# nikisalli/nightmare_rl

Measured on AMD Instinct MI355X. Metric: env-steps/sec at N parallel Nightmare-v3 envs, 1/2/4/8 MI355X, higher is better.
Workload: dtype f32; 1 GPU; 4096 Nightmare-v3 envs per GPU, random-action rollout U(-1,1)^18, full step(): 2 x 8 ms substeps (18-DoF dynamics + floor contact, PGS x3 + noslip x4) + obs/reward/termination/reset; envs_per_gpu=4096, decimation=2

## Files before the change

### nightmare_rl_amd/csrc/nm_core.h

```cpp
#pragma once
#include <type_traits>
#include <stddef.h>

#include "simt.h"

#ifdef NM_MEASURE
#define NM_ABLATE(mask) (mask)
#else
#define NM_ABLATE(mask) 0
#endif
namespace nm {
using namespace simt;

constexpr int kNQ = 25, kNV = 24, kNU = 18, kNLEG = 6, kNCOL = 7, kNSENS = 13, kNOBS = 66, kNREW = 16;
constexpr int kLinkN = 25;
constexpr int kLegN = 3 * kLinkN;
constexpr int kBaseN = 10;
constexpr int kColN = 24;
constexpr int kMaxCon = 16;
constexpr int kMaxRow = 4 * kMaxCon;
constexpr int kMaxConBig = 44;
constexpr int kBigSlots = (4 * kMaxConBig + NM_WAVE - 1) / NM_WAVE;
constexpr int kJRow = 16;
enum { R_ACTION_RATE, R_ANG_VEL_XY, R_BASE_HEIGHT, R_BODY_CONTACT, R_DEFAULT_POS, R_DOF_ACC, R_DOF_VEL, R_FEET_AIR_TIME, R_FEET_CONTACT,
       R_LIN_VEL_Z, R_ORIENTATION, R_STAND_STILL, R_TORQUES, R_TRACK_ANG, R_TRACK_LIN, R_TERMINATION };

template <class real> struct Model {
  const real* hullv;
  const real* hullnv;
  real legc[kNLEG * kLegN];
  real basec[kBaseN];
  real colc[kNCOL * kColN];
  real footc[kNLEG * 4];
  real qpos0[kNQ];
  int maxnbr;
  int link_rot_id[3];
  real total_mass;
  real h, kv, ctrl_max, grav, mu;
  real solref_K, solref_B, si_d0, si_dmax, si_width, si_mid, si_power;
  real pgs_scale, pgs_tol, noslip_tol, tol_planemesh;
  int pgs_iters, noslip_iters, mpr_iters;
  real mpr_tol;
  real dt, p_gain, clip_obs, obs_lin, obs_ang, obs_dofpos, obs_dofvel, max_lin_x, max_ang, term_force, sigma, max_ep_len, default_pos[3];
  float action_scale, clip_actions;
  int resample_every;
  real rew_scale[kNREW];
  real ep_len_s;
  int rew_extra;
  int tibia_mode, body_mode;
  int collide_batch_min;
  real tibia_max, body_max, base_h_target, max_contact_force;
};

template <class real> struct Args {
  int N;
  int rec_env;
  uint64_t seed;
  int64_t env_offset;
  real *qpos, *qvel, *qwarm;
  real *dofpos, *dofvel, *act, *cmd, *epsum;
  real* feetair;
  int* feetflags;
  int64_t* eplen;
  uint32_t* rngctr;
  int* hullcache;
  const float* actions;
  const real* cmd_u;
  float *obs, *rew, *timeout_now;
  float* ret_acc;
  int64_t* done;
  real* stat_sum;
  int* stat_cnt;
  int* wave_done;
  int *nto, *to_list;
  int *nprev, *to_prev;
  unsigned long long* to_owner;
  float *ep_stats, *time_outs;
  long long* counters;
  real* dbg;
  int nsub;
  int nxcd;
  int physics_only;
  int ablate;
  const real* noise_vec;
  const real* noise_u;
  uint64_t noise_step;
  real* rec;
  const real* envp;
};
constexpr int kTicketGroup = 64, kTicketStride = 32, kTicketTop = 0;
constexpr uint64_t kNoiseKey = 0x4E4F495345ull;
constexpr uint64_t kEnvParamKey = 0x454E5650ull;
constexpr int EP_MU = 0, EP_PGAIN = 1, EP_KV = 2, kEnvP = 4, kEnvPS = 3;
constexpr int kBodyP = 20, BP_IPOS = 0, BP_I6 = 3, BP_MASS = 9, BP_TOTAL = 10, BP_INVW = 11, BP_PGS = 18;
constexpr uint64_t kPayloadKey = 0x5041594C4Full;
constexpr int kLatH = 3, kLatP = 1 + kLatH * 18;
constexpr uint64_t kLatencyKey = 0x4C4154454Eull;
template <class real> NM_FN int* lat_delay(const Args<real>& A) {
  return reinterpret_cast<int*>(const_cast<real*>(A.envp) + (size_t)A.N * (kEnvP + kBodyP));
}
template <class real> NM_FN float* lat_hist(const Args<real>& A) { return reinterpret_cast<float*>(lat_delay(A) + A.N); }
constexpr int kDbgN = 256;

template <class real> struct Sh {
  real qpos[kNQ];
  real envp[kEnvPS];
  real qvel[24], warm[24], ctrl[20];
  real Rb[9], wv[6];
  real anc[kNU * 3], axs[kNU * 3];
  real colR[kNCOL * 9], colp[kNCOL * 3];
  real Minv[kNLEG * 6], W[kNLEG * 18], Lb[15], Dbi[6];
  real MinvH[kNLEG * 6], WH[kNLEG * 18], LbH[15], DbiH[6];
  real qas[24], qfs[24], qfc[24];
  real vv[24];
  real sens[16], cvb[6];
  real bh[2];
  real mbb[36], sc[36];
  real legtmp[kNLEG * 66];
  NM_FN real* cpos() { return legtmp; }
  NM_FN real* cnrm() { return legtmp + 3 * kMaxConBig; }
  NM_FN real* cdist() { return legtmp + 6 * kMaxConBig; }
  NM_FN int* cleg() { return reinterpret_cast<int*>(legtmp + 7 * kMaxConBig); }
  NM_FN int* cleg1() { return reinterpret_cast<int*>(legtmp + 8 * kMaxConBig); }
  real efc_f[kMaxRow];
#ifdef NM_DEBUG_SOLVER
  real dbg_b[kMaxRow], dbg_a[kMaxRow], dbg_f0[kMaxRow];
#endif
  int ncon, nwarn, it_pgs, it_noslip, anypair;
  int nhop;
  int ntog;
  real eact[kNU], epact[kNU], epdv[kNU];
  real ecmd[4], eepsum[kNREW];
  int eplen_lo, eplen_hi;
  unsigned ectr;
  int cstart[8], ccnt[8];
  real sink[NM_WAVE];
  int hcache[8];
};

static_assert(kNLEG * 66 >= 9 * kMaxConBig, "contact list must fit the leg staging area");
static_assert(offsetof(Sh<float>, qvel) == 28 * sizeof(float) && offsetof(Sh<double>, qvel) == 28 * sizeof(double), "qpos + envp keep the 28 words qpos had");
template <class real, int G> struct ShW {
  Sh<real> e[G];
  alignas(16) real jrow[kMaxRow * kJRow];
};
template <class real, int G> struct ShWB {
  ShW<real, G> w;
  real body[G * kBodyP];
};
template <class real, int G> NM_FN real* body_rows(ShW<real, G>& w) { return reinterpret_cast<ShWB<real, G>*>(&w)->body; }
template <class real, int G, int EP> struct ShWSel {
  typedef ShW<real, G> type;
  static NM_FN ShW<real, G>& images(type& s) { return s; }
};
template <class real, int G> struct ShWSel<real, G, 2> {
  typedef ShWB<real, G> type;
  static NM_FN ShW<real, G>& images(type& s) { return s.w; }
};
template <class real, int G> struct ShWL {
  ShWB<real, G> b;
  real late[G * 18];
  int rsw[G];
};
template <class real, int G> NM_FN ShWL<real, G>& lat_rows(ShW<real, G>& w) { return *reinterpret_cast<ShWL<real, G>*>(&w); }
template <class real, int G> struct ShWSel<real, G, 3> {
  typedef ShWL<real, G> type;
  static NM_FN ShW<real, G>& images(type& s) { return s.b.w; }
};
#define NM_OFS(field) ((int)(offsetof(Sh<real>, field) / sizeof(real)))
#define NM_IOFS(field) ((int)(offsetof(Sh<real>, field) / sizeof(int)))

template <int EP, class real> NM_FN real env_mu(const Sh<real>& sh, const Model<real>& M) {
  if constexpr (EP != 0) return sh.envp[EP_MU]; else return M.mu;
}
template <int EP, class real> struct BodyRef {
  NM_FN BodyRef() {}
  NM_FN explicit BodyRef(const real*) {}
};
template <class real> struct BodyRef<2, real> {
  const real* p;
  NM_FN BodyRef() : p(nullptr) {}
  NM_FN explicit BodyRef(const real* q) : p(q) {}
};
template <class real> struct BodyRef<3, real> {
  const real* p;
  NM_FN BodyRef() : p(nullptr) {}
  NM_FN explicit BodyRef(const real* q) : p(q) {}
};
template <int EP, class real> NM_FN V<real> body_invw(const BodyRef<EP, real>& b, const Model<real>& M, const V<int>& g) {
  if constexpr (EP >= 2) return ldsv(b.p, g + BP_INVW); else return ldsv(M.colc, g * kColN + 4);
}
template <int EP, class real> NM_FN real body_pgs(const BodyRef<EP, real>& b, const Model<real>& M) {
  if constexpr (EP >= 2) return b.p[BP_PGS]; else return M.pgs_scale;
}

template <class A, class B, class C> NM_FN void cross3(A* r, const B* a, const C* b) {
  A x = a[1] * b[2] - a[2] * b[1], y = a[2] * b[0] - a[0] * b[2], z = a[0] * b[1] - a[1] * b[0];
  r[0] = x; r[1] = y; r[2] = z;
}
template <class A, class B, class C> NM_FN A dot3(const B* a, const C* b) { return a[0] * b[0] + a[1] * b[1] + a[2] * b[2]; }
template <class A, class B, class C> NM_FN void matvec3(A* r, const B* m, const C* v) {
  A x = m[0] * v[0] + m[1] * v[1] + m[2] * v[2], y = m[3] * v[0] + m[4] * v[1] + m[5] * v[2], z = m[6] * v[0] + m[7] * v[1] + m[8] * v[2];
  r[0] = x; r[1] = y; r[2] = z;
}
template <class A, class B, class C> NM_FN void matvec3_fma(A* r, const B* m, const C* v) {
  A x = vfma(A(m[2]), A(v[2]), vfma(A(m[1]), A(v[1]), A(m[0]) * A(v[0])));
  A y = vfma(A(m[5]), A(v[2]), vfma(A(m[4]), A(v[1]), A(m[3]) * A(v[0])));
  A z = vfma(A(m[8]), A(v[2]), vfma(A(m[7]), A(v[1]), A(m[6]) * A(v[0])));
  r[0] = x; r[1] = y; r[2] = z;
}
template <class A, class B, class C> NM_FN void matmul3(A* r, const B* a, const C* b) {
#pragma unroll
  for (int i = 0; i < 3; i++)
#pragma unroll
    for (int j = 0; j < 3; j++) r[3 * i + j] = a[3 * i] * b[j] + a[3 * i + 1] * b[3 + j] + a[3 * i + 2] * b[6 + j];
}
template <class A, class B, class C> NM_FN void inert_mul(A* r, const B* i, const C* v) {
  r[0] = i[0] * v[0] + i[3] * v[1] + i[4] * v[2] - i[8] * v[4] + i[7] * v[5];
  r[1] = i[3] * v[0] + i[1] * v[1] + i[5] * v[2] + i[8] * v[3] - i[6] * v[5];
  r[2] = i[4] * v[0] + i[5] * v[1] + i[2] * v[2] - i[7] * v[3] + i[6] * v[4];
  r[3] = i[8] * v[1] - i[7] * v[2] + i[9] * v[3];
  r[4] = i[6] * v[2] - i[8] * v[0] + i[9] * v[4];
  r[5] = i[7] * v[0] - i[6] * v[1] + i[9] * v[5];
}
template <class A, class B, class C> NM_FN void cross_motion(A* r, const B* vel, const C* v) {
  A a[3], b[3], c[3];
  cross3(a, vel, v); cross3(b, vel, v + 3); cross3(c, vel + 3, v);
  r[0] = a[0]; r[1] = a[1]; r[2] = a[2]; r[3] = b[0] + c[0]; r[4] = b[1] + c[1]; r[5] = b[2] + c[2];
}
template <class A, class B, class C> NM_FN void cross_force(A* r, const B* vel, const C* f) {
  A a[3], b[3], c[3];
  cross3(a, vel, f); cross3(b, vel + 3, f + 3); cross3(c, vel, f + 3);
  r[0] = a[0] + b[0]; r[1] = a[1] + b[1]; r[2] = a[2] + b[2]; r[3] = c[0]; r[4] = c[1]; r[5] = c[2];
}
template <class A, class B, class C> NM_FN A dot6(const B* a, const C* b) {
  return a[0] * b[0] + a[1] * b[1] + a[2] * b[2] + a[3] * b[3] + a[4] * b[4] + a[5] * b[5];
}
template <class real> NM_FN real lanesum6(const V<real>& x) {
  return ((rdlane(x, 0) + rdlane(x, 1)) + (rdlane(x, 2) + rdlane(x, 3))) + (rdlane(x, 4) + rdlane(x, 5));
}
template <class X, class real> NM_FN void spatial_inertia(X* I10, const X* R, const X* Ib, const X* d, X m, real) {
  X T[9];
#pragma unroll
  for (int i = 0; i < 3; i++) {
    T[3 * i + 0] = R[3 * i] * Ib[0] + R[3 * i + 1] * Ib[3] + R[3 * i + 2] * Ib[4];
    T[3 * i + 1] = R[3 * i] * Ib[3] + R[3 * i + 1] * Ib[1] + R[3 * i + 2] * Ib[5];
    T[3 * i + 2] = R[3 * i] * Ib[4] + R[3 * i + 1] * Ib[5] + R[3 * i + 2] * Ib[2];
  }
  X xx = T[0] * R[0] + T[1] * R[1] + T[2] * R[2], yy = T[3] * R[3] + T[4] * R[4] + T[5] * R[5], zz = T[6] * R[6] + T[7] * R[7] + T[8] * R[8];
  X xy = T[0] * R[3] + T[1] * R[4] + T[2] * R[5], xz = T[0] * R[6] + T[1] * R[7] + T[2] * R[8], yz = T[3] * R[6] + T[4] * R[7] + T[5] * R[8];
  I10[0] = xx + m * (d[1] * d[1] + d[2] * d[2]);
  I10[1] = yy + m * (d[0] * d[0] + d[2] * d[2]);
  I10[2] = zz + m * (d[0] * d[0] + d[1] * d[1]);
  I10[3] = xy - m * d[0] * d[1];
  I10[4] = xz - m * d[0] * d[2];
  I10[5] = yz - m * d[1] * d[2];
  I10[6] = m * d[0]; I10[7] = m * d[1]; I10[8] = m * d[2];
  I10[9] = m;
}
template <class X, class real> NM_FN void ldl3(X* r, const X* a, real one) {
  X i2 = vrcp(a[5]);
  X l21 = a[4] * i2, l20 = a[2] * i2;
  X m11 = a[3] - l21 * a[4], m01 = a[1] - l21 * a[2], m00 = a[0] - l20 * a[2];
  X i1 = vrcp(m11);
  X l10 = m01 * i1;
  X d0 = m00 - l10 * m01;
  r[0] = l21; r[1] = l20; r[2] = l10; r[3] = i2; r[4] = i1; r[5] = vrcp(d0);
}
template <class X, class Y> NM_FN void ldl3_solve(X* x, const X* f, const Y* y) {
  X y2 = y[2];
  X y1 = y[1] - f[0] * y2;
  X y0 = y[0] - f[1] * y2 - f[2] * y1;
  X x0 = y0 * f[5];
  X x1 = y1 * f[4] - f[2] * x0;
  x[2] = y2 * f[3] - f[0] * x1 - f[1] * x0;
  x[1] = x1; x[0] = x0;
}
template <class X, class real, class Acc> NM_FN void ldl6(Acc S, X* L, X* Dinv, real one) {
  X Lf[36], D[6];
#pragma unroll
  for (int j = 0; j < 6; j++) {
    X d = S(j, j);
#pragma unroll
    for (int k = 0; k < j; k++) d = d - Lf[6 * j + k] * Lf[6 * j + k] * D[k];
    D[j] = d;
    X di = vrcp(d);
    Dinv[j] = di;
#pragma unroll
    for (int i = j + 1; i < 6; i++) {
      X s = S(j, i);
#pragma unroll
      for (int k = 0; k < j; k++) s = s - Lf[6 * i + k] * Lf[6 * j + k] * D[k];
      Lf[6 * i + j] = s * di;
    }
  }
  int n = 0;
#pragma unroll
  for (int i = 1; i < 6; i++)
#pragma unroll
    for (int j = 0; j < i; j++) L[n++] = Lf[6 * i + j];
}
template <class LT, class X> NM_FN void ldl6_solve(const LT* L, const LT* Dinv, X* x) {
  int n = 0;
#pragma unroll
  for (int i = 1; i < 6; i++)
#pragma unroll
    for (int j = 0; j < i; j++) x[i] = x[i] - L[n++] * x[j];
#pragma unroll
  for (int i = 0; i < 6; i++) x[i] = x[i] * Dinv[i];
#pragma unroll
  for (int i = 5; i >= 1; i--) {
    n = i * (i - 1) / 2;
#pragma unroll
    for (int j = 0; j < i; j++) x[j] = x[j] - L[n + j] * x[i];
  }
}

NM_HDFN uint32_t rand_u24_bits(uint64_t seed, uint64_t genv, uint32_t ctr) {
  uint64_t x = seed + 0x9E3779B97F4A7C15ull * (genv + 1) + 0xD1B54A32D192ED03ull * (uint64_t)ctr;
  x ^= x >> 30; x *= 0xBF58476D1CE4E5B9ull;
  x ^= x >> 27; x *= 0x94D049BB133111EBull;
  x ^= x >> 31;
  return (uint32_t)(x >> 40);
}

#ifndef NM_EMUL
template <class T> NM_FN void nm_consume(T x) { asm volatile("" ::"v"(x) : "memory"); }
#endif

#if defined(NM_STAMPS) && !defined(NM_EMUL)
__device__ unsigned long long g_stamps[16];
NM_FN void nm_stamp(int k) {
  __shared__ unsigned long long tl, acc[16];
#ifdef NM_STAMPS_B
  asm volatile("s_waitcnt vmcnt(0) lgkmcnt(0)" ::: "memory");
#endif
  unsigned long long n = __builtin_amdgcn_s_memtime();
  if (NM_TID == 0) {
    if (k < 0) for (int i = 0; i < 16; i++) acc[i] = 0;
    else acc[k] += n - tl;
    if (k == 10) for (int i = 0; i < 16; i++) atomicAdd(&g_stamps[i], acc[i]);
    tl = n;
  }
}
#else
NM_FN void nm_stamp(int) {}
#endif
#ifdef NM_STAMPS_B
#define NM_ESTAMP(k)
#define NM_BSTAMP(k) nm_stamp(k)
#else
#define NM_ESTAMP(k) nm_stamp(k)
#define NM_BSTAMP(k)
#endif

constexpr int kLinkTmp = 22;

template <class real> NM_FN V<real> legsum(const V<real>& x, const VB& isleg) {
  return gsum8(sel(isleg, x, V<real>(real(0))));
}

template <int EP, class real, int G> NM_FN void stage_smooth(ShW<real, G>& w, const Model<real>& M, bool last) {
  typedef V<real> vr;
  real* lds = reinterpret_cast<real*>(&w.e[0]);
  static_assert((G & (G - 1)) == 0 && 2 * G <= 8, "lane groups: G envs x 2 factorisations");
  const V<int> lane0 = opaque_lane();
  const V<int> sub = lane0 & 7, grp = lane0 >> 3;
  const V<int> leg = vmin(sub, V<int>(5)), eo = (grp & (G - 1)) * (int)(sizeof(Sh<real>) / sizeof(real));
  const VB pass1 = (grp & G) != 0;
  const VB isleg = sub < V<int>(6);
#define LDG(field, i) ldsv(lds, eo + (NM_OFS(field) + (i)))
  const V<int> bo = (grp & (G - 1)) * kBodyP + (int)(sizeof(ShW<real, G>) / sizeof(real));
#define LDB(i) ldsv(lds, bo + (i))
  const VB st_all = VB(true), st_leg = VB(true);
#define STG(field, i, val) stsv(lds, eo + (NM_OFS(field) + (i)), val, st_all)
#define LDL(field, idx) ldsv(lds, eo + (idx) + NM_OFS(field))
#define STL(field, idx, val) stsv(lds, eo + (idx) + NM_OFS(field), val, st_leg)
  const V<int> slot = leg * (3 * kLinkTmp);

  vr Rb[9];
  {
    vr qw = LDG(qpos, 3), qx = LDG(qpos, 4), qy = LDG(qpos, 5), qz = LDG(qpos, 6);
    {
      const vr in_ = vrcp(vsqrt(qw * qw + qx * qx + qy * qy + qz * qz));
      qw = qw * in_; qx = qx * in_; qy = qy * in_; qz = qz * in_;
      STG(qpos, 3, qw); STG(qpos, 4, qx); STG(qpos, 5, qy); STG(qpos, 6, qz);
    }
    vr q00 = qw * qw, q01 = qw * qx, q02 = qw * qy, q03 = qw * qz, q11 = qx * qx, q12 = qx * qy, q13 = qx * qz, q22 = qy * qy,
       q23 = qy * qz, q33 = qz * qz;
    Rb[0] = q00 + q11 - q22 - q33; Rb[4] = q00 - q11 + q22 - q33; Rb[8] = q00 - q11 - q22 + q33;
    Rb[1] = real(2) * (q12 - q03); Rb[2] = real(2) * (q13 + q02); Rb[3] = real(2) * (q12 + q03);
    Rb[5] = real(2) * (q23 - q01); Rb[6] = real(2) * (q13 - q02); Rb[7] = real(2) * (q23 + q01);
  }
  vr vb[6], ab[6];
  {
    vr wl[3] = {LDG(qvel, 3), LDG(qvel, 4), LDG(qvel, 5)};
    matvec3(vb, Rb, wl);
    vb[3] = LDG(qvel, 0); vb[4] = LDG(qvel, 1); vb[5] = LDG(qvel, 2);
    vr t[3];
    cross3(t, vb + 3, vb);
    ab[0] = ab[1] = ab[2] = vr(real(0));
    ab[3] = t[0]; ab[4] = t[1]; ab[5] = t[2] + M.grav;
  }
#pragma unroll
  for (int j = 0; j < 9; j++) { STG(colR, j, Rb[j]); STG(Rb, j, Rb[j]); }
#pragma unroll
// ... 2306 lines not shown
    sh.eplen_hi = (int)(ep >> 32);
    sh.ectr = ctr_in;
    if constexpr (EP == 3) {
      const int nsub = A.nsub;
      const int k = (dl >= nsub ? 1 : 0) + (dl >= 2 * nsub ? 1 : 0) + (dl >= 3 * nsub ? 1 : 0), r = dl - k * nsub;
      const V<float> fl = k == 0 ? af : (k == 1 ? h0 : (k == 2 ? h1 : h2));
      const V<float> fe = r > 0 ? (k == 0 ? h0 : (k == 1 ? h1 : h2)) : fl;
      stsv(sh.ctrl, lane, ((vcvt<real>(fe) - defp) - dofpos_old) * p_gain, l18);
      stsv(late, lane, ((vcvt<real>(fl) - defp) - dofpos_old) * p_gain, l18);
      *rsw = r;
      float* hist = lat_hist(A);
      const VB st = l18 & VB(live);
      gstv(hist, lane + (env * (kLatH * kNU) + 2 * kNU), h1, st);
      gstv(hist, lane + (env * (kLatH * kNU) + kNU), h0, st);
      gstv(hist, lane + env * (kLatH * kNU), af, st);
    } else
    stsv(sh.ctrl, lane, ((act - defp) - dofpos_old) * p_gain, l18);
  } else {
    wave_sync();
    stsv(sh.ctrl, lane, ((act - defp) - ldsv(sh.qpos, l18c + 7)) * p_gain, l18);
    if constexpr (EP == 3) *rsw = 0;
  }
  stsv(sh.eact, lane, act, l18); stsv(sh.epact, lane, prev_act, l18); stsv(sh.epdv, lane, prev_dofvel, l18);
  wave_sync();
}

template <class real> NM_FN void env_debug(Sh<real>& sh, const Args<real>& A, int env, int dropped) {
  const V<int> lane = opaque_lane();
  {
    real* dbg = A.dbg + (size_t)env * kDbgN;
    gstv(dbg, lane, ldsv(sh.qas, sel(lane < 24, lane, V<int>(0))), lane < 24);
    gstv(dbg, lane + 24, ldsv(sh.qfs, sel(lane < 24, lane, V<int>(0))), lane < 24);
    gstv(dbg, lane + 48, ldsv(sh.qfc, sel(lane < 24, lane, V<int>(0))), lane < 24);
    gstv(dbg, lane + 72, ldsv(sh.sens, sel(lane < 13, lane, V<int>(0))), lane < 13);
    gstv(dbg, lane + 88, ldsv(sh.cvb, sel(lane < 6, lane, V<int>(0))), lane < 6);
    gstv(dbg, lane + 96, ldsv(sh.cdist(), sel(lane < kMaxCon, lane, V<int>(0))), lane < kMaxCon);
    gstv(dbg, lane + 112, ldsv(sh.cpos(), sel(lane < 3 * kMaxCon, lane, V<int>(0))), lane < 3 * kMaxCon);
    gstv(dbg, V<int>(160), to_real<real>(sh.ncon), lane == 0);
    gstv(dbg, V<int>(161), to_real<real>(sh.nwarn), lane == 0);
    gstv(dbg, V<int>(162), to_real<real>(dropped), lane == 0);
    gstv(dbg, lane + 165, ldsv(sh.cnrm(), sel(lane < 6, lane, V<int>(0))), lane < 6);
    gstv(dbg, lane + 150, to_real<real>(ldsv(sh.hcache, sel(lane < 7, lane, V<int>(0)))), lane < 7);
    gstv(dbg, V<int>(158), to_real<real>(sh.hcache[7]), lane == 0);
    gstv(dbg, V<int>(159), to_real<real>(sh.nhop), lane == 0);
    gstv(dbg, V<int>(157), to_real<real>(sh.anypair), lane == 0);
    gstv(dbg, V<int>(156), to_real<real>(sh.ntog), lane == 0);
    gstv(dbg, V<int>(163), to_real<real>(sh.it_pgs), lane == 0);
    gstv(dbg, V<int>(164), to_real<real>(sh.it_noslip), lane == 0);
    gstv(dbg, lane + 176, ldsv(sh.efc_f, lane), lane < kMaxRow);
#ifdef NM_DEBUG_SOLVER
    gstv(dbg, lane + 240, ldsv(sh.dbg_b, sel(lane < 4, lane, V<int>(0))), lane < 4);
    gstv(dbg, lane + 244, ldsv(sh.dbg_a, sel(lane < 4, lane, V<int>(0))), lane < 4);
    gstv(dbg, lane + 248, ldsv(sh.dbg_f0, sel(lane < 4, lane, V<int>(0))), lane < 4);
#endif
  }
}

template <class real> NM_FN void env_finish(Sh<real>& sh, const Model<real>& M, const Args<real>& A, int env,
                                            int dropped, bool live) {
  typedef V<real> vr;
  if (!live) return;
  const V<int> lane = opaque_lane();
  const VB l18 = lane < kNU;
  const V<int> l18c = sel(l18, lane, V<int>(0));
  const vr act = ldsv(sh.eact, l18c), prev_act = ldsv(sh.epact, l18c), prev_dofvel = ldsv(sh.epdv, l18c);
  vr defp;
  {
    V<int> m3 = lane % 3;
    defp = sel(m3 == 1, vr(M.default_pos[1]), sel(m3 == 0, vr(M.default_pos[0]), vr(M.default_pos[2])));
  }
  {
    const V<int> hc = ldsv(sh.hcache, sel(lane < 8, lane, V<int>(0)));
    const vr q = ldsv(sh.qpos, sel(lane < kNQ, lane, V<int>(0))), v = ldsv(sh.qvel, sel(lane < kNV, lane, V<int>(0))),
             w = ldsv(sh.warm, sel(lane < kNV, lane, V<int>(0)));
    gstv(A.hullcache, lane + env * 8, hc, lane < 8);
    gstv(A.qpos, lane + env * kNQ, q, lane < kNQ);
    gstv(A.qvel, lane + env * kNV, v, lane < kNV);
    gstv(A.qwarm, lane + env * kNV, w, lane < kNV);
  }
  if (A.rec && env == A.rec_env) {
    gstv(A.rec, lane, ldsv(sh.qpos, sel(lane < kNQ, lane, V<int>(0))), lane < kNQ);
    gstv(A.rec, lane + kNQ, ldsv(sh.qvel, sel(lane < kNV, lane, V<int>(0))), lane < kNV);
    gstv(A.rec, V<int>(kNQ + kNV), to_real<real>(sh.nwarn), lane == 0);
  }
  if (A.dbg) env_debug(sh, A, env, dropped);
  if ((dropped | sh.nwarn) && A.stat_cnt) {
#ifdef NM_EMUL
    A.stat_cnt[1] += dropped; A.stat_cnt[2] += sh.nwarn;
#else
    if (NM_TID == 0) { nm_consume(atomicAdd(A.stat_cnt + 1, dropped)); nm_consume(atomicAdd(A.stat_cnt + 2, sh.nwarn)); }
#endif
  }
  if (A.physics_only) return;
  NM_ESTAMP(11);

  int64_t eplen = (((int64_t)sh.eplen_hi << 32) | (int64_t)(uint32_t)sh.eplen_lo) + 1;
  real bq[4] = {sh.qpos[3], -sh.qpos[4], -sh.qpos[5], -sh.qpos[6]};
  auto rot = [&](real* r, const real* v) {
    real tx = real(2) * (bq[2] * v[2] - bq[3] * v[1]), ty = real(2) * (bq[3] * v[0] - bq[1] * v[2]), tz = real(2) * (bq[1] * v[1] - bq[2] * v[0]);
    r[0] = v[0] + bq[0] * tx + (bq[2] * tz - bq[3] * ty);
    r[1] = v[1] + bq[0] * ty + (bq[3] * tx - bq[1] * tz);
    r[2] = v[2] + bq[0] * tz + (bq[1] * ty - bq[2] * tx);
  };
  real blv[3], bav[3], pg[3];
  {
    real lin[3] = {sh.cvb[3], sh.cvb[4], sh.cvb[5]}, ang[3] = {sh.cvb[0], sh.cvb[1], sh.cvb[2]}, gv[3] = {real(0), real(0), -M.grav};
    rot(blv, lin); rot(bav, ang); rot(pg, gv);
  }
  vr dofpos = ldsv(sh.qpos, l18c + 7), dofvel = ldsv(sh.qvel, l18c + 6);
  real tib[6], feet[6], body = sh.sens[12];
#pragma unroll
  for (int l = 0; l < 6; l++) {
    feet[l] = sh.sens[6 + l];
    tib[l] = feet[l] == real(0) ? sh.sens[l] : real(0);
  }
  real cmd[3] = {sh.ecmd[0], sh.ecmd[1], sh.ecmd[2]};
  uint32_t ctr = sh.ectr;
  auto resample = [&](int which) {
    real ux, uy;
    if (A.cmd_u) { ux = gld1(A.cmd_u, env * 4 + 2 * which); uy = gld1(A.cmd_u, env * 4 + 2 * which + 1); }
    else {
      ux = (real)rand_u24_bits(A.seed, (uint64_t)(A.env_offset + env), ctr) * real(1.0 / 16777216.0);
      uy = (real)rand_u24_bits(A.seed, (uint64_t)(A.env_offset + env), ctr + 1) * real(1.0 / 16777216.0);
      ctr += 2;
    }
    cmd[0] = ux * real(2) * M.max_lin_x - M.max_lin_x;
    cmd[1] = real(0);
    cmd[2] = uy * real(2) * M.max_ang - M.max_ang;
    real keep = vsqrt(cmd[0] * cmd[0] + cmd[1] * cmd[1]) > real(0.02) ? real(1) : real(0);
    cmd[0] = cmd[0] * keep; cmd[1] = cmd[1] * keep;
  };
  {
    bool due;
    if (eplen >= 0 && eplen < (1 << 22)) {
      const int e32 = (int)eplen, R = M.resample_every;
      const int q = (int)((float)e32 / (float)R);
      const int r = e32 - q * R;
      due = r == 0 || r == R || r == -R;
    } else due = eplen % M.resample_every == 0;
    if (due) resample(0);
  }
  bool time_out = (real)eplen > M.max_ep_len;
  bool reset = time_out;
  {
    real fm = feet[0];
#pragma unroll
    for (int l = 1; l < 6; l++) fm = vmax(fm, feet[l]);
    reset = reset | (fm > M.term_force);
    if ((M.tibia_mode == 2) | (M.body_mode == 2)) {
      real tm = tib[0];
#pragma unroll
      for (int l = 1; l < 6; l++) tm = vmax(tm, tib[l]);
      if (M.tibia_mode == 2) reset = reset | (tm > M.tibia_max);
      if (M.body_mode == 2) reset = reset | (body > M.body_max);
    }
    real nrm = vsqrt(pg[0] * pg[0] + pg[1] * pg[1] + pg[2] * pg[2]);
    if (sizeof(real) == 8) reset = reset | (vacos(-pg[2] / nrm) > real(1.0471975511965976));
    else reset = reset | (-pg[2] / nrm <= real(0.5));
  }
  NM_ESTAMP(12);
  vr epsum[1];
  V<int> l8c = sel(lane < kNREW, lane, V<int>(0));
  epsum[0] = ldsv(sh.eepsum, l8c);
  if (reset) {
    gstv(A.qpos, lane + env * kNQ, ldsv(M.qpos0, sel(lane < kNQ, lane, V<int>(0))), lane < kNQ);
    gstv(A.qvel, lane + env * kNV, real(0), lane < kNV);
    resample(1);
    eplen = 0;
#ifdef NM_EMUL
    for (int k = 0; k < kNREW; k++) A.stat_sum[k] += epsum[0].v[k];
    A.stat_cnt[0] += 1;
#else
    if (NM_TID < kNREW) nm_consume(atomicAdd(A.stat_sum + NM_TID, epsum[0]));
    if (NM_TID == 0) {
      nm_consume(atomicAdd(A.stat_cnt, 1));
      if (time_out && A.to_list) nm_consume(atomicExch(A.to_list + atomicAdd(A.nto, 1), env));
    }
#endif
    epsum[0] = vr(real(0));
  }
  NM_ESTAMP(13);
  real rt[kNREW];
#pragma unroll
  for (int k = 0; k < kNREW; k++) rt[k] = real(0);
  {
    vr da = prev_act - act;
    rt[R_ACTION_RATE] = wsum<real>(sel(l18, da * da, vr(real(0)))) * M.rew_scale[R_ACTION_RATE];
    real sumt = ((tib[0] + tib[1]) + (tib[2] + tib[3])) + (tib[4] + tib[5]);
    if ((M.tibia_mode != 1) | (M.body_mode != 1)) {
      sumt = M.tibia_mode == 1 ? sumt : real(0);
      body = M.body_mode == 1 ? body : real(0);
    }
    rt[R_BODY_CONTACT] = (sumt + body) * M.rew_scale[R_BODY_CONTACT];
    vr dp = dofpos - defp;
    rt[R_DEFAULT_POS] = wsum<real>(sel(l18, dp * dp, vr(real(0)))) * M.rew_scale[R_DEFAULT_POS];
    vr acc = (dofvel - prev_dofvel) / M.dt;
    rt[R_DOF_ACC] = wsum<real>(sel(l18, acc * acc, vr(real(0)))) * M.rew_scale[R_DOF_ACC];
    rt[R_ORIENTATION] = (pg[0] * pg[0] + pg[1] * pg[1]) * M.rew_scale[R_ORIENTATION];
    real ea = (cmd[2] - bav[2]) * (cmd[2] - bav[2]);
    rt[R_TRACK_ANG] = vexp(-ea / M.sigma) * M.rew_scale[R_TRACK_ANG];
    real el = (cmd[0] - blv[0]) * (cmd[0] - blv[0]) + (cmd[1] - blv[1]) * (cmd[1] - blv[1]);
    rt[R_TRACK_LIN] = vexp(-el / M.sigma) * M.rew_scale[R_TRACK_LIN];
    rt[R_TERMINATION] = (reset && !time_out) ? M.rew_scale[R_TERMINATION] : real(0);
    if (M.rew_extra) {
      rt[R_ANG_VEL_XY] = (bav[0] * bav[0] + bav[1] * bav[1]) * M.rew_scale[R_ANG_VEL_XY];
      real dh = sh.bh[0] - M.base_h_target;
      rt[R_BASE_HEIGHT] = dh * dh * M.rew_scale[R_BASE_HEIGHT];
      rt[R_DOF_VEL] = wsum<real>(sel(l18, dofvel * dofvel, vr(real(0)))) * M.rew_scale[R_DOF_VEL];
      rt[R_LIN_VEL_Z] = blv[2] * blv[2] * M.rew_scale[R_LIN_VEL_Z];
      real still = vsqrt(cmd[0] * cmd[0] + cmd[1] * cmd[1]) < real(0.01) ? real(1) : real(0);
      rt[R_STAND_STILL] = wsum<real>(sel(l18, vabs(dp), vr(real(0)))) * still * M.rew_scale[R_STAND_STILL];
      const VB l6 = lane < kNLEG;
      const V<int> l6c = sel(l6, lane, V<int>(0));
      const vr ff = ldsv(sh.sens, l6c + 6);
      vr over = sel(ff > vr(M.max_contact_force), ff - M.max_contact_force, vr(real(0)));
      rt[R_FEET_CONTACT] = wsum<real>(sel(l6, over * over, vr(real(0)))) * M.rew_scale[R_FEET_CONTACT];
      if (M.rew_scale[R_FEET_AIR_TIME] != real(0)) {
        vr air = gldv(A.feetair, l6c + env * kNLEG);
        const V<int> fl = V<int>(gld1(A.feetflags, env));
        if (reset) air = vr(real(0));
        const VB contact = ff > vr(real(1));
        const VB filt = contact | (((fl >> l6c) & 1) != 0);
        const VB lastf = ((fl >> (l6c + kNLEG)) & 1) != 0;
        air = air + M.dt;
        air = sel(filt == lastf, air, vr(real(0)));
        const vr single = sel(air > vr(real(1)), air - real(1), vr(real(0))) + sel(air < vr(real(0.5)), real(0.5) - air, vr(real(0)));
        rt[R_FEET_AIR_TIME] = wsum<real>(sel(l6, single * single, vr(real(0)))) * M.rew_scale[R_FEET_AIR_TIME];
        gstv(A.feetair, l6c + env * kNLEG, air, l6);
        const int nf = (int)(ballot(l6 & contact) | (ballot(l6 & filt) << kNLEG));
#ifdef NM_EMUL
        A.feetflags[env] = nf;
#else
        if (NM_TID == 0) gst1(A.feetflags, env, nf);
#endif
      }
    }
  }
  real rew = real(0);
#pragma unroll
  for (int k = 0; k < kNREW; k++) rew = rew + rt[k];
  {
    vr add = vr(real(0));
#pragma unroll
    for (int k = 0; k < kNREW; k++) add = wrlane(add, rt[k], k);
    gstv(A.epsum, lane + env * kNREW, epsum[0] + add, lane < kNREW);
  }
  NM_ESTAMP(14);
  {
    real head[12] = {blv[0] * M.obs_lin, blv[1] * M.obs_lin, blv[2] * M.obs_lin, bav[0] * M.obs_ang, bav[1] * M.obs_ang, bav[2] * M.obs_ang,
                     pg[0], pg[1], pg[2], cmd[0] * M.obs_lin, cmd[1] * M.obs_lin, cmd[2] * M.obs_ang};
    vr o = vr(real(0));
#pragma unroll
    for (int k = 0; k < 12; k++) o = wrlane(o, head[k], k);
    auto put = [&](const vr& x0, const V<int>& idx, const VB& m) {
      vr x = x0;
      if (A.noise_vec) {
        auto nz = [&](int k) {
          real u = A.noise_u ? gld1(A.noise_u, (size_t)env * kNOBS + k)
                             : (real)rand_u24_bits(A.seed + kNoiseKey, (uint64_t)(A.env_offset + env), (uint32_t)(A.noise_step * kNOBS + k)) * real(1.0 / 16777216.0);
          return (real(2) * u - real(1)) * gld1(A.noise_vec, k);
        };
#ifdef NM_EMUL
        for (int i = 0; i < NM_WAVE; i++) if (m.v[i]) x.v[i] = x.v[i] + nz(idx.v[i]);
#else
        if (m) x = x + nz(idx);
#endif
      }
      vr cx = vmin(vmax(x, vr(-M.clip_obs)), vr(M.clip_obs));
#ifdef NM_EMUL
      for (int i = 0; i < NM_WAVE; i++) if (m.v[i]) A.obs[(size_t)env * kNOBS + idx.v[i]] = (float)cx.v[i];
#else
      if (m) gst1(A.obs, (size_t)env * kNOBS + idx, (float)cx);
#endif
    };
    put(o, lane, lane < 12);
    put((dofpos - defp) * M.obs_dofpos, lane + 12, l18);
    put(dofvel * M.obs_dofvel, lane + 30, l18);
    put(act, lane + 48, l18);
  }
  NM_ESTAMP(15);
  gstv(A.dofpos, lane + env * kNU, dofpos, l18);
  gstv(A.dofvel, lane + env * kNU, dofvel, l18);
  gstv(A.act, lane + env * kNU, act, l18);
  {
    vr cv = sel(lane == 0, vr(cmd[0]), sel(lane == 1, vr(cmd[1]), vr(cmd[2])));
    gstv(A.cmd, lane + env * 3, cv, lane < 3);
  }
#ifdef NM_EMUL
  const bool lane0 = true;
#else
  const bool lane0 = NM_TID == 0;
#endif
  if (lane0) {
    gst1(A.eplen, env, eplen);
    gst1(A.rngctr, env, ctr);
    gst1(A.rew, env, (float)rew);
    if (A.ret_acc) gadd1(A.ret_acc, env, (float)rew);
    gst1(A.done, env, (int64_t)(reset ? 1 : 0));
    gst1(A.timeout_now, env, time_out ? 1.0f : 0.0f);
  }
}

struct NoMid { NM_FN void operator()() const {} NM_FN void operator()(int) const {} };
template <int EP, class real, class Mid> NM_FN void env_load2(ShW<real, 2>& w, const Model<real>& M, const Args<real>& A, int wave, Mid&& mid) {
  typedef V<real> vr;
  constexpr int kSR = (int)(sizeof(Sh<real>) / sizeof(real)), kSI = (int)(sizeof(Sh<real>) / sizeof(int));
  const V<int> lane = opaque_lane();
  const V<int> h = lane >> 5, hl = lane & 31;
  const V<int> env0 = h + wave * 2;
  const V<int> env = sel(env0 < V<int>(A.N), env0, V<int>(A.N - 1));
  real* rb = reinterpret_cast<real*>(&w.e[0]);
  int* ib = reinterpret_cast<int*>(&w.e[0]);
  const V<int> ho = h * kSR, hoi = h * kSI;
  const VB l18 = hl < kNU;
  const V<int> l18c = sel(l18, hl, V<int>(0));
  const vr q_in = gldv(A.qpos, sel(hl < kNQ, hl, V<int>(0)) + env * kNQ);
  const vr v_in = gldv(A.qvel, sel(hl < kNV, hl, V<int>(0)) + env * kNV);
  const vr w_in = gldv(A.qwarm, sel(hl < kNV, hl, V<int>(0)) + env * kNV);
  const V<int> hc_in = gldv(A.hullcache, sel(hl < 8, hl, V<int>(0)) + env * 8);
  const V<float> a_in = gldv(A.actions, l18c + env * kNU);
  vr envp_in = vr(real(0));
  if constexpr (EP != 0) envp_in = gldv(A.envp, sel(hl < kEnvP, hl, V<int>(0)) + env * kEnvP);
  vr body_in = vr(real(0));
  if constexpr (EP >= 2) body_in = gldv(A.envp, sel(hl < kBodyP, hl, V<int>(0)) + (env * kBodyP + A.N * kEnvP));
  vr cmd_in = vr(real(0)), eps_in = vr(real(0)), prev_act = vr(real(0)), prev_dofvel = vr(real(0)), dofpos_old = vr(real(0));
  V<int> dl = V<int>(0);
  V<float> h0 = V<float>(0.0f), h1 = V<float>(0.0f), h2 = V<float>(0.0f);
  if constexpr (EP == 3)
    if (!A.physics_only) {
      dl = gldv(lat_delay(A), env);
      h0 = gldv(lat_hist(A), l18c + env * (kLatH * kNU));
      h1 = gldv(lat_hist(A), l18c + (env * (kLatH * kNU) + kNU));
      h2 = gldv(lat_hist(A), l18c + (env * (kLatH * kNU) + 2 * kNU));
    }
#ifndef NM_EMUL
  int64_t ep = 0;
  uint32_t ctr_in = 0;
#endif
  if (!A.physics_only) {
    cmd_in = gldv(A.cmd, sel(hl < 3, hl, V<int>(0)) + env * 3);
    eps_in = gldv(A.epsum, sel(hl < kNREW, hl, V<int>(0)) + env * kNREW);
#ifndef NM_EMUL
    ep = gld1(A.eplen, (size_t)env);
    ctr_in = gld1(A.rngctr, (size_t)env);
#endif
    prev_act = gldv(A.act, l18c + env * kNU);
    prev_dofvel = gldv(A.dofvel, l18c + env * kNU);
    dofpos_old = gldv(A.dofpos, l18c + env * kNU);
  }
  mid();
  stsv(rb, ho + (hl + NM_OFS(qpos)), q_in, hl < kNQ);
  stsv(rb, ho + (hl + NM_OFS(qvel)), v_in, hl < kNV);
  stsv(rb, ho + (hl + NM_OFS(warm)), w_in, hl < kNV);
  stsv(ib, hoi + (hl + NM_IOFS(hcache)), sel(hl == 0, hc_in & V<int>(0xffff), hc_in), hl < 8);
  nm_set_priority((rdlane(hc_in, 0) >> 16) + (rdlane(hc_in, 32) >> 16));
  w.e[0].nwarn = 0; w.e[1].nwarn = 0;
  w.e[0].nhop = 0; w.e[1].nhop = 0;
  w.e[0].ntog = 0; w.e[1].ntog = 0;
  vr p_gain = vr(M.p_gain);
  if constexpr (EP != 0) {
    stsv(rb, ho + (hl + NM_OFS(envp)), envp_in, hl < kEnvPS);
    if constexpr (EP >= 2) stsv(body_rows(w), h * kBodyP + hl, body_in, hl < kBodyP);
    p_gain = sel(h != 0, vr(rdlane(envp_in, 32 + EP_PGAIN)), vr(rdlane(envp_in, EP_PGAIN)));
  }
  V<float> af = a_in * M.action_scale;
  af = vmin(vmax(af, V<float>(-M.clip_actions)), V<float>(M.clip_actions));
  vr act;
  vr defp;
  {
    V<int> m3 = hl % 3;
    defp = sel(m3 == 1, vr(M.default_pos[1]), sel(m3 == 0, vr(M.default_pos[0]), vr(M.default_pos[2])));
  }
#ifdef NM_EMUL
  for (int i = 0; i < NM_WAVE; i++) act.v[i] = (real)af.v[i];
#else
  act = (real)af;
#endif
  if (!A.physics_only) {
    stsv(rb, ho + (hl + NM_OFS(ecmd)), cmd_in, hl < 3);
    stsv(rb, ho + (hl + NM_OFS(eepsum)), eps_in, hl < kNREW);
#ifdef NM_EMUL
    for (int hh = 0; hh < 2; hh++) {
      const int e = env.v[32 * hh];
      const int64_t ep = A.eplen[e];
      w.e[hh].eplen_lo = (int)(uint32_t)(ep & 0xffffffffll);
      w.e[hh].eplen_hi = (int)(ep >> 32);
      w.e[hh].ectr = A.rngctr[e];
    }
#else
    stsv(ib, hoi + NM_IOFS(eplen_lo), (int)(uint32_t)(ep & 0xffffffffll), hl == 0);
    stsv(ib, hoi + NM_IOFS(eplen_hi), (int)(ep >> 32), hl == 0);
    stsv(ib, hoi + NM_IOFS(ectr), (int)ctr_in, hl == 0);
#endif
    if constexpr (EP == 3) {
      const V<int> ns = V<int>(A.nsub), one = V<int>(1), zero = V<int>(0);
      const V<int> k = sel(dl >= ns, one, zero) + sel(dl >= ns + ns, one, zero) + sel(dl >= ns + ns + ns, one, zero), r = dl - k * ns;
      const V<float> fl = sel(k == zero, af, sel(k == one, h0, sel(k == V<int>(2), h1, h2)));
      const V<float> fe = sel(r > zero, sel(k == zero, h0, sel(k == one, h1, h2)), fl);
      ShWL<real, 2>& L = lat_rows(w);
      stsv(rb, ho + (hl + NM_OFS(ctrl)), ((vcvt<real>(fe) - defp) - dofpos_old) * p_gain, l18);
      stsv(L.late, h * kNU + hl, ((vcvt<real>(fl) - defp) - dofpos_old) * p_gain, l18);
      stsv(L.rsw, h, r, hl == zero);
      float* hist = lat_hist(A);
      const VB st = l18 & (env0 < V<int>(A.N));
      gstv(hist, hl + (env * (kLatH * kNU) + 2 * kNU), h1, st);
      gstv(hist, hl + (env * (kLatH * kNU) + kNU), h0, st);
      gstv(hist, hl + env * (kLatH * kNU), af, st);
    } else
    stsv(rb, ho + (hl + NM_OFS(ctrl)), ((act - defp) - dofpos_old) * p_gain, l18);
  } else {
    wave_sync();
    stsv(rb, ho + (hl + NM_OFS(ctrl)), ((act - defp) - ldsv(rb, ho + (l18c + (7 + NM_OFS(qpos))))) * p_gain, l18);
    if constexpr (EP == 3) stsv(lat_rows(w).rsw, h, V<int>(0), hl == V<int>(0));
  }
  stsv(rb, ho + (hl + NM_OFS(eact)), act, l18); stsv(rb, ho + (hl + NM_OFS(epact)), prev_act, l18); stsv(rb, ho + (hl + NM_OFS(epdv)), prev_dofvel, l18);
  wave_sync();
}

template <class real, class Pub> NM_FN void env_finish2(ShW<real, 2>& w, const Model<real>& M, const Args<real>& A, int wave, int dropped, Pub&& published) {
  typedef V<real> vr;
  constexpr int kSR = (int)(sizeof(Sh<real>) / sizeof(real)), kSI = (int)(sizeof(Sh<real>) / sizeof(int));
  const V<int> lane = opaque_lane();
  const V<int> h = lane >> 5, hl = lane & 31;
  const VB h1 = h != 0;
  const V<int> env = h + wave * 2;
  const VB live = env < V<int>(A.N);
  const V<int> envc = sel(live, env, V<int>(A.N - 1));
  const bool lives[2] = {wave * 2 < A.N, wave * 2 + 1 < A.N};
  const real* rb = reinterpret_cast<const real*>(&w.e[0]);
  const int* ib = reinterpret_cast<const int*>(&w.e[0]);
  const V<int> ho = h * kSR, hoi = h * kSI;
#define SHR(field, idx) ldsv(rb, ho + ((idx) + NM_OFS(field)))
#define SHI(field, idx) ldsv(ib, hoi + ((idx) + NM_IOFS(field)))
  const VB l18 = hl < kNU;
  const V<int> l18c = sel(l18, hl, V<int>(0));
  const vr act = SHR(eact, l18c), prev_act = SHR(epact, l18c), prev_dofvel = SHR(epdv, l18c);
  vr defp;
  {
    V<int> m3 = hl % 3;
    defp = sel(m3 == 1, vr(M.default_pos[1]), sel(m3 == 0, vr(M.default_pos[0]), vr(M.default_pos[2])));
  }
  const V<int> nwarn = SHI(nwarn, V<int>(0));
  {
    V<int> hc = SHI(hcache, sel(hl < 8, hl, V<int>(0)));
    hc = sel(hl == 0, hc | (SHI(ncon, V<int>(0)) << 16), hc);
    const vr q = SHR(qpos, sel(hl < kNQ, hl, V<int>(0))), v = SHR(qvel, sel(hl < kNV, hl, V<int>(0))), wq = SHR(warm, sel(hl < kNV, hl, V<int>(0)));
    gstv(A.hullcache, hl + env * 8, hc, live & (hl < 8));
    gstv(A.qpos, hl + env * kNQ, q, live & (hl < kNQ));
    gstv(A.qvel, hl + env * kNV, v, live & (hl < kNV));
    gstv(A.qwarm, hl + env * kNV, wq, live & (hl < kNV));
    if (A.rec) {
      const VB r = live & (env == V<int>(A.rec_env));
      gstv(A.rec, hl, q, r & (hl < kNQ));
      gstv(A.rec, hl + kNQ, v, r & (hl < kNV));
      gstv(A.rec, V<int>(kNQ + kNV), to_real<real>(nwarn), r & (hl == 0));
    }
  }
  if (A.dbg) {
    if (lives[0]) env_debug(w.e[0], A, wave * 2, dropped);
    if (lives[1]) env_debug(w.e[1], A, wave * 2 + 1, 0);
  }
  if (A.stat_cnt && (dropped != 0 || wany(live & (nwarn != 0)))) {
#ifdef NM_EMUL
    A.stat_cnt[1] += dropped;
    for (int hh = 0; hh < 2; hh++) if (lives[hh]) A.stat_cnt[2] += nwarn.v[32 * hh];
#else
    if (NM_TID == 0 && dropped) nm_consume(atomicAdd(A.stat_cnt + 1, dropped));
    if (hl == 0 && live && nwarn) nm_consume(atomicAdd(A.stat_cnt + 2, nwarn));
#endif
  }
  if (A.physics_only) return;
  if (NM_ABLATE(A.ablate) & 128) return;
  NM_ESTAMP(11);

  int64_t ep[2];
  uint32_t ctr[2];
#pragma unroll
  for (int hh = 0; hh < 2; hh++) {
    ep[hh] = (((int64_t)w.e[hh].eplen_hi << 32) | (int64_t)(uint32_t)w.e[hh].eplen_lo) + 1;
    ctr[hh] = w.e[hh].ectr;
  }
  vr bq[4] = {SHR(qpos, V<int>(3)), -SHR(qpos, V<int>(4)), -SHR(qpos, V<int>(5)), -SHR(qpos, V<int>(6))};
  auto rot = [&](vr* r, const vr* v) {
    vr tx = real(2) * (bq[2] * v[2] - bq[3] * v[1]), ty = real(2) * (bq[3] * v[0] - bq[1] * v[2]), tz = real(2) * (bq[1] * v[1] - bq[2] * v[0]);
    r[0] = v[0] + bq[0] * tx + (bq[2] * tz - bq[3] * ty);
    r[1] = v[1] + bq[0] * ty + (bq[3] * tx - bq[1] * tz);
    r[2] = v[2] + bq[0] * tz + (bq[1] * ty - bq[2] * tx);
  };
  vr blv[3], bav[3], pg[3];
  {
    vr lin[3] = {SHR(cvb, V<int>(3)), SHR(cvb, V<int>(4)), SHR(cvb, V<int>(5))}, ang[3] = {SHR(cvb, V<int>(0)), SHR(cvb, V<int>(1)), SHR(cvb, V<int>(2))};
    vr gv[3] = {vr(real(0)), vr(real(0)), vr(-M.grav)};
    rot(blv, lin); rot(bav, ang); rot(pg, gv);
  }
  vr dofpos = SHR(qpos, l18c + 7), dofvel = SHR(qvel, l18c + 6);
  vr tib[6], feet[6], body = SHR(sens, V<int>(12));
#pragma unroll
  for (int l = 0; l < 6; l++) {
    feet[l] = SHR(sens, V<int>(6 + l));
    tib[l] = sel(feet[l] == vr(real(0)), SHR(sens, V<int>(l)), vr(real(0)));
  }
  vr cmd[3] = {SHR(ecmd, V<int>(0)), SHR(ecmd, V<int>(1)), SHR(ecmd, V<int>(2))};
  auto resample = [&](int hh, int which) {
    const int e = wave * 2 + hh;
    real ux, uy;
    if (A.cmd_u) { ux = gld1(A.cmd_u, (size_t)(e * 4 + 2 * which)); uy = gld1(A.cmd_u, (size_t)(e * 4 + 2 * which + 1)); }
    else {
      ux = (real)rand_u24_bits(A.seed, (uint64_t)(A.env_offset + e), ctr[hh]) * real(1.0 / 16777216.0);
      uy = (real)rand_u24_bits(A.seed, (uint64_t)(A.env_offset + e), ctr[hh] + 1) * real(1.0 / 16777216.0);
      ctr[hh] += 2;
    }
    real c0 = ux * real(2) * M.max_lin_x - M.max_lin_x, c1 = real(0), c2 = uy * real(2) * M.max_ang - M.max_ang;
    real keep = vsqrt(c0 * c0 + c1 * c1) > real(0.02) ? real(1) : real(0);
    c0 = c0 * keep; c1 = c1 * keep;
    const VB mine = hh ? h1 : !h1;
    cmd[0] = sel(mine, vr(c0), cmd[0]); cmd[1] = sel(mine, vr(c1), cmd[1]); cmd[2] = sel(mine, vr(c2), cmd[2]);
  };
  bool tos[2];
#pragma unroll
  for (int hh = 0; hh < 2; hh++) {
    bool due;
    if (ep[hh] >= 0 && ep[hh] < (1 << 22)) {
      const int e32 = (int)ep[hh], R = M.resample_every;
      const int q = (int)((float)e32 / (float)R);
      const int r = e32 - q * R;
      due = r == 0 || r == R || r == -R;
    } else due = ep[hh] % M.resample_every == 0;
    if (due && lives[hh]) resample(hh, 0);
    tos[hh] = (real)ep[hh] > M.max_ep_len;
  }
  const VB time_out = (h1 & VB(tos[1])) | (!h1 & VB(tos[0]));
  VB reset = time_out;
  {
    vr fm = feet[0];
#pragma unroll
    for (int l = 1; l < 6; l++) fm = vmax(fm, feet[l]);
    reset = reset | (fm > vr(M.term_force));
    if ((M.tibia_mode == 2) | (M.body_mode == 2)) {
      vr tm = tib[0];
#pragma unroll
      for (int l = 1; l < 6; l++) tm = vmax(tm, tib[l]);
      if (M.tibia_mode == 2) reset = reset | (tm > vr(M.tibia_max));
      if (M.body_mode == 2) reset = reset | (body > vr(M.body_max));
    }
    vr nrm = vsqrt(pg[0] * pg[0] + pg[1] * pg[1] + pg[2] * pg[2]);
    if (sizeof(real) == 8) reset = reset | (vacos(-pg[2] / nrm) > vr(real(1.0471975511965976)));
    else reset = reset | ((-pg[2] / nrm) <= vr(real(0.5)));
  }
  NM_ESTAMP(12);
  vr epsum = SHR(eepsum, sel(hl < kNREW, hl, V<int>(0)));
  const VB resetL = reset & live;
  const uint64_t rmask = ballot(resetL);
  if (rmask) {
    gstv(A.qpos, hl + env * kNQ, ldsv(M.qpos0, sel(hl < kNQ, hl, V<int>(0))), resetL & (hl < kNQ));
    gstv(A.qvel, hl + env * kNV, real(0), resetL & (hl < kNV));
#pragma unroll
    for (int hh = 0; hh < 2; hh++)
      if ((rmask >> (32 * hh)) & 1) { resample(hh, 1); ep[hh] = 0; }
#ifdef NM_EMUL
    for (int hh = 0; hh < 2; hh++)
      if ((rmask >> (32 * hh)) & 1) {
        for (int k = 0; k < kNREW; k++) A.stat_sum[k] += epsum.v[32 * hh + k];
        A.stat_cnt[0] += 1;
      }
#else
    if (resetL && hl < kNREW) nm_consume(atomicAdd(A.stat_sum + hl, epsum));
    if (resetL && hl == 0) {
      nm_consume(atomicAdd(A.stat_cnt, 1));
      if (time_out && A.to_list) nm_consume(atomicExch(A.to_list + atomicAdd(A.nto, 1), env));
    }
#endif
    epsum = sel(resetL, vr(real(0)), epsum);
  }
  published(0);
  NM_ESTAMP(13);
  vr rt[kNREW];
#pragma unroll
  for (int k = 0; k < kNREW; k++) rt[k] = vr(real(0));
  {
    vr da = prev_act - act;
    rt[R_ACTION_RATE] = hsum32(sel(l18, da * da, vr(real(0)))) * M.rew_scale[R_ACTION_RATE];
    vr sumt = ((tib[0] + tib[1]) + (tib[2] + tib[3])) + (tib[4] + tib[5]);
    if ((M.tibia_mode != 1) | (M.body_mode != 1)) {
      sumt = M.tibia_mode == 1 ? sumt : vr(real(0));
      body = M.body_mode == 1 ? body : vr(real(0));
    }
    rt[R_BODY_CONTACT] = (sumt + body) * M.rew_scale[R_BODY_CONTACT];
    vr dp = dofpos - defp;
    rt[R_DEFAULT_POS] = hsum32(sel(l18, dp * dp, vr(real(0)))) * M.rew_scale[R_DEFAULT_POS];
    vr acc = (dofvel - prev_dofvel) / M.dt;
    rt[R_DOF_ACC] = hsum32(sel(l18, acc * acc, vr(real(0)))) * M.rew_scale[R_DOF_ACC];
    rt[R_ORIENTATION] = (pg[0] * pg[0] + pg[1] * pg[1]) * M.rew_scale[R_ORIENTATION];
    vr ea = (cmd[2] - bav[2]) * (cmd[2] - bav[2]);
    rt[R_TRACK_ANG] = vexp(-ea / M.sigma) * M.rew_scale[R_TRACK_ANG];
    vr el = (cmd[0] - blv[0]) * (cmd[0] - blv[0]) + (cmd[1] - blv[1]) * (cmd[1] - blv[1]);
    rt[R_TRACK_LIN] = vexp(-el / M.sigma) * M.rew_scale[R_TRACK_LIN];
    rt[R_TERMINATION] = sel(reset & !time_out, vr(M.rew_scale[R_TERMINATION]), vr(real(0)));
    if (M.rew_extra) {
      rt[R_ANG_VEL_XY] = (bav[0] * bav[0] + bav[1] * bav[1]) * M.rew_scale[R_ANG_VEL_XY];
      vr dh = SHR(bh, V<int>(0)) - M.base_h_target;
      rt[R_BASE_HEIGHT] = dh * dh * M.rew_scale[R_BASE_HEIGHT];
      rt[R_DOF_VEL] = hsum32(sel(l18, dofvel * dofvel, vr(real(0)))) * M.rew_scale[R_DOF_VEL];
      rt[R_LIN_VEL_Z] = blv[2] * blv[2] * M.rew_scale[R_LIN_VEL_Z];
      vr still = sel(vsqrt(cmd[0] * cmd[0] + cmd[1] * cmd[1]) < vr(real(0.01)), vr(real(1)), vr(real(0)));
      rt[R_STAND_STILL] = hsum32(sel(l18, vabs(dp), vr(real(0)))) * still * M.rew_scale[R_STAND_STILL];
      const VB l6 = hl < kNLEG;
      const V<int> l6c = sel(l6, hl, V<int>(0));
      const vr ff = SHR(sens, l6c + 6);
      vr over = sel(ff > vr(M.max_contact_force), ff - M.max_contact_force, vr(real(0)));
      rt[R_FEET_CONTACT] = hsum32(sel(l6, over * over, vr(real(0)))) * M.rew_scale[R_FEET_CONTACT];
      if (M.rew_scale[R_FEET_AIR_TIME] != real(0)) {
        vr air = gldv(A.feetair, l6c + envc * kNLEG);
        const V<int> fl = gldv(A.feetflags, envc);
        air = sel(reset, vr(real(0)), air);
        const VB contact = ff > vr(real(1));
        const VB filt = contact | (((fl >> l6c) & 1) != 0);
        const VB lastf = ((fl >> (l6c + kNLEG)) & 1) != 0;
        air = air + M.dt;
        air = sel(filt == lastf, air, vr(real(0)));
        const vr single = sel(air > vr(real(1)), air - real(1), vr(real(0))) + sel(air < vr(real(0.5)), real(0.5) - air, vr(real(0)));
        rt[R_FEET_AIR_TIME] = hsum32(sel(l6, single * single, vr(real(0)))) * M.rew_scale[R_FEET_AIR_TIME];
        gstv(A.feetair, l6c + env * kNLEG, air, live & l6);
        const uint64_t bc = ballot(l6 & contact), bf = ballot(l6 & filt);
        const int nf0 = (int)((bc & 63) | ((bf & 63) << kNLEG)), nf1 = (int)(((bc >> 32) & 63) | (((bf >> 32) & 63) << kNLEG));
        gstv(A.feetflags, env, sel(h1, V<int>(nf1), V<int>(nf0)), live & (hl == 0));
      }
    }
  }
  vr rew = vr(real(0));
#pragma unroll
  for (int k = 0; k < kNREW; k++) rew = rew + rt[k];
  {
    vr add = vr(real(0));
#pragma unroll
    for (int k = 0; k < kNREW; k++) add = sel(hl == k, rt[k], add);
    gstv(A.epsum, hl + env * kNREW, epsum + add, live & (hl < kNREW));
  }
  published(1);
  NM_ESTAMP(14);
  if (!(NM_ABLATE(A.ablate) & 256)) {
    vr head[12] = {blv[0] * M.obs_lin, blv[1] * M.obs_lin, blv[2] * M.obs_lin, bav[0] * M.obs_ang, bav[1] * M.obs_ang, bav[2] * M.obs_ang,
                   pg[0], pg[1], pg[2], cmd[0] * M.obs_lin, cmd[1] * M.obs_lin, cmd[2] * M.obs_ang};
    vr o = vr(real(0));
#pragma unroll
    for (int k = 0; k < 12; k++) o = sel(hl == k, head[k], o);
    auto put = [&](const vr& x0, const V<int>& idx, const VB& m0) {
      const VB m = m0 & live;
      vr x = x0;
      if (A.noise_vec) {
        auto nz = [&](int k, int e) {
          real u = A.noise_u ? gld1(A.noise_u, (size_t)e * kNOBS + k)
                             : (real)rand_u24_bits(A.seed + kNoiseKey, (uint64_t)(A.env_offset + e), (uint32_t)(A.noise_step * kNOBS + k)) * real(1.0 / 16777216.0);
          return (real(2) * u - real(1)) * gld1(A.noise_vec, (size_t)k);
        };
#ifdef NM_EMUL
        for (int i = 0; i < NM_WAVE; i++) if (m.v[i]) x.v[i] = x.v[i] + nz(idx.v[i], env.v[i]);
#else
        if (m) x = x + nz(idx, env);
#endif
      }
      vr cx = vmin(vmax(x, vr(-M.clip_obs)), vr(M.clip_obs));
#ifdef NM_EMUL
      for (int i = 0; i < NM_WAVE; i++) if (m.v[i]) A.obs[(size_t)env.v[i] * kNOBS + idx.v[i]] = (float)cx.v[i];
#else
      if (m) gst1(A.obs, (size_t)env * kNOBS + idx, (float)cx);
#endif
    };
    put(o, hl, hl < 12);
    put((dofpos - defp) * M.obs_dofpos, hl + 12, l18);
    put(dofvel * M.obs_dofvel, hl + 30, l18);
    put(act, hl + 48, l18);
  }
  NM_ESTAMP(15);
  gstv(A.dofpos, hl + env * kNU, dofpos, live & l18);
  gstv(A.dofvel, hl + env * kNU, dofvel, live & l18);
  gstv(A.act, hl + env * kNU, act, live & l18);
  {
    vr cv = sel(hl == 0, cmd[0], sel(hl == 1, cmd[1], cmd[2]));
    gstv(A.cmd, hl + env * 3, cv, live & (hl < 3));
  }
#ifdef NM_EMUL
  for (int hh = 0; hh < 2; hh++)
    if (lives[hh]) {
      const int e = wave * 2 + hh, l0 = 32 * hh;
      A.eplen[e] = ep[hh]; A.rngctr[e] = ctr[hh]; A.rew[e] = (float)rew.v[l0];
      if (A.ret_acc) A.ret_acc[e] += (float)rew.v[l0];
      A.done[e] = (int64_t)(reset.v[l0] ? 1 : 0); A.timeout_now[e] = time_out.v[l0] ? 1.0f : 0.0f;
    }
#else
  if (hl == 0 && live) {
    gst1(A.eplen, (size_t)env, h1 ? ep[1] : ep[0]);
    gst1(A.rngctr, (size_t)env, h1 ? ctr[1] : ctr[0]);
    gst1(A.rew, (size_t)env, (float)rew);
    if (A.ret_acc) gadd1(A.ret_acc, (size_t)env, (float)rew);
    gst1(A.done, (size_t)env, (int64_t)(reset ? 1 : 0));
    gst1(A.timeout_now, (size_t)env, time_out ? 1.0f : 0.0f);
  }
#endif
#undef SHR
#undef SHI
}

template <class real, int G> NM_FN void latency_switch(ShW<real, G>& w, int s) {
  ShWL<real, G>& L = lat_rows(w);
  const V<int> lane = opaque_lane();
  wave_sync();
  if constexpr (G == 2) {
    constexpr int kSR = (int)(sizeof(Sh<real>) / sizeof(real));
    real* rb = reinterpret_cast<real*>(&w.e[0]);
    const V<int> h = lane >> 5, hl = lane & 31;
    const VB on = (hl < kNU) & (ldsv(L.rsw, h) == V<int>(s));
    const V<real> cmd = ldsv(L.late, h * kNU + sel(hl < kNU, hl, V<int>(0)));
    stsv(rb, h * kSR + (hl + NM_OFS(ctrl)), cmd, on);
  } else {
    for (int e = 0; e < G; e++)
      if (uniform(L.rsw[e]) == s) stsv(w.e[e].ctrl, lane, ldsv(L.late, sel(lane < kNU, lane, V<int>(0)) + e * kNU), lane < kNU);
  }
  wave_sync();
}

template <class real, int G, int EP = 0, class Mid = NoMid, class Pub = NoMid>
NM_FN void wave_step(ShW<real, G>& w, const Model<real>& M, const Args<real>& A, int wave, Mid&& mid = Mid(), Pub&& published = Pub()) {
  nm_stamp(-1);
  if constexpr (G == 2) {
    env_load2<EP>(w, M, A, wave, mid);
  } else {
    mid();
#pragma unroll
    for (int e = 0; e < G; e++) {
      int env = wave * G + e;
      real* bp = nullptr;
      if constexpr (EP >= 2) bp = body_rows(w) + e * kBodyP;
      if constexpr (EP == 3) env_load<EP>(w.e[e], M, A, env < A.N ? env : A.N - 1, bp, lat_rows(w).late + e * kNU, lat_rows(w).rsw + e, env < A.N);
      else
      env_load<EP>(w.e[e], M, A, env < A.N ? env : A.N - 1, bp);
    }
  }
  nm_stamp(0);
  int dropped = 0;
  if (NM_ABLATE(A.ablate) & 1024) return;
  if (!(NM_ABLATE(A.ablate) & 2048))
  for (int s = 0; s < A.nsub; s++) {
    if constexpr (EP == 3) { if (s > 0) latency_switch(w, s); }
    substep<EP>(w, M, s == A.nsub - 1, &dropped, NM_ABLATE(A.ablate));
  }
  if constexpr (G == 2) {
    env_finish2(w, M, A, wave, dropped, published);
  } else {
#pragma unroll
    for (int e = 0; e < G; e++) {
      int env = wave * G + e;
      env_finish(w.e[e], M, A, env, e == 0 ? dropped : 0, env < A.N);
    }
  }
  nm_stamp(10);
}

}
```

### nightmare_rl_amd/csrc/nm_hip.hip

```cpp
#include <hip/hip_runtime.h>

#include <cmath>
#include <cstdio>
#include <cstdlib>
#include <cstring>
#include <string>
#include <vector>

#include "../../include/nightmare_hip.h"
#include "nm_host_model.h"
#include "nm_env_loop.h"
#include "nm_env_rows.h"
#include "nm_push.h"
#include "nm_reset_noise.h"
#include "nm_rollout.h"

static thread_local std::string g_err;
static int fail(const std::string& m) { g_err = m; return 1; }
#define HIPCHK(x)                                                                                        \
  do {                                                                                                   \
    hipError_t e_ = (x);                                                                                 \
    if (e_ != hipSuccess) return fail(std::string(#x) + ": " + hipGetErrorString(e_));                  \
  } while (0)

#ifndef NM_WAVES_PER_SIMD
#define NM_WAVES_PER_SIMD 2
#endif
#ifndef NM_ENVS_PER_WAVE
#define NM_ENVS_PER_WAVE 2
#endif
template <class real> __device__ __noinline__ void step_tail(const nm::Args<real>& A, real ep_len_s) {
  const int lane = NM_TID;
#define TAIL_LD(p) __hip_atomic_load(p, __ATOMIC_RELAXED, __HIP_MEMORY_SCOPE_AGENT)
  const int cnt = TAIL_LD(A.stat_cnt);
  const int c1 = TAIL_LD(A.stat_cnt + 1), c2 = TAIL_LD(A.stat_cnt + 2);
  const real ssum = TAIL_LD(A.stat_sum + (lane < nm::kNREW ? lane : 0));
  const int n = TAIL_LD(A.nto);
  const int np = TAIL_LD(A.nprev);
  const bool to_full = A.time_outs && TAIL_LD(A.to_owner) != (unsigned long long)(uintptr_t)A.time_outs;
  const long long k0 = lane == 0 ? A.counters[0] : 0, k1 = lane == 0 ? A.counters[1] : 0;
  if (cnt > 0) {
    if (lane < nm::kNREW && A.ep_stats) A.ep_stats[lane] = (float)(ssum / (real)cnt / ep_len_s);
    if (A.time_outs) {
      const int e_new = lane < n ? TAIL_LD(A.to_list + lane) : -1;
      const int e_old = (!to_full && lane < np) ? A.to_prev[lane] : -1;
      if (to_full) {
        for (int i = lane; i < A.N; i += 64) A.time_outs[i] = 0.f;
      } else {
        if (e_old >= 0) A.time_outs[e_old] = 0.f;
        for (int j = lane + 64; j < np; j += 64) A.time_outs[A.to_prev[j]] = 0.f;
      }
      asm volatile("s_waitcnt vmcnt(0)" ::: "memory");
      if (e_new >= 0) { A.time_outs[e_new] = 1.f; A.to_prev[lane] = e_new; }
      for (int j = lane + 64; j < n; j += 64) {
        const int e = TAIL_LD(A.to_list + j);
        A.time_outs[e] = 1.f;
        A.to_prev[j] = e;
      }
      if (lane == 0) { *A.nprev = n; *A.to_owner = (unsigned long long)(uintptr_t)A.time_outs; }
    }
  }
#undef TAIL_LD
  if (lane < nm::kNREW) A.stat_sum[lane] = real(0);
  if (lane == 0) {
    A.counters[0] = k0 + c1;
    A.counters[1] = k1 + c2;
    A.stat_cnt[0] = 0; A.stat_cnt[1] = 0; A.stat_cnt[2] = 0; A.stat_cnt[3] = 0;
    *A.nto = 0;
    A.wave_done[nm::kTicketTop] = 0;
  }
}

#ifdef NM_WG_WAVES
constexpr int kWG = NM_WG_WAVES;
#else
constexpr int kWG = 1;
#endif
template <class real, int G, int EP>
__global__ void __launch_bounds__(64 * (sizeof(real) == 8 ? 1 : kWG), NM_WAVES_PER_SIMD) k_env_step(const nm::Model<real>* __restrict__ Mp, nm::Args<real> A) {
  constexpr int kWG = sizeof(real) == 8 ? 1 : ::kWG;
  __shared__ typename nm::ShWSel<real, G, EP>::type shs[kWG];
  __shared__ nm::Model<real> Ms;
  __shared__ nm::Args<real> As;
  nm::ShW<real, G>& sh = nm::ShWSel<real, G, EP>::images(shs[kWG == 1 ? 0 : (int)(threadIdx.x >> 6)]);
  int wave = nmr::wave_index(A.nxcd);
  if (kWG > 1) wave = wave * kWG + (int)(threadIdx.x >> 6);
#ifdef NM_MEASURE
  if (A.ablate & 512) return;
#endif
  const unsigned long long t_start = A.dbg ? __builtin_amdgcn_s_memtime() : 0ull;
  if (kWG == 1 || threadIdx.x < 64) As = A;
  __syncthreads();
  if (wave * G >= A.N) return;
  auto copy_model = [&]() {
    const uint32_t* src = reinterpret_cast<const uint32_t*>(Mp);
    uint32_t* dst = reinterpret_cast<uint32_t*>(&Ms);
    constexpr int kWords = (int)(sizeof(nm::Model<real>) / 4);
    uint32_t tmp[(kWords + 63) / 64];
#pragma unroll
    for (int k = 0; k < (kWords + 63) / 64; k++) { const int i = NM_TID + 64 * k; tmp[k] = i < kWords ? src[i] : 0u; }
    if (kWG == 1 || threadIdx.x < 64) {
#pragma unroll
      for (int k = 0; k < (kWords + 63) / 64; k++) { const int i = NM_TID + 64 * k; if (i < kWords) dst[i] = tmp[k]; }
    }
    __syncthreads();
  };
  const int nw = (As.N + G - 1) / G, grp = wave / nm::kTicketGroup, ngrp = (nw + nm::kTicketGroup - 1) / nm::kTicketGroup;
  const int gsize = min(nm::kTicketGroup, nw - grp * nm::kTicketGroup);
  int ticket = 0, top = 0;
  int stage = 0;
  bool closes_group = false;
  auto draw = [&](int phase) {
#ifdef NM_NO_TICKETS
    stage = 2; (void)phase; return;
#endif
    if (phase == 0) {
      if (NM_TID == 0) ticket = atomicAdd(As.wave_done + (grp + 1) * nm::kTicketStride, 1);
      stage = 1;
    } else {
      closes_group = __builtin_amdgcn_readfirstlane(ticket) == gsize - 1;
      if (closes_group && NM_TID == 0) {
        As.wave_done[(grp + 1) * nm::kTicketStride] = 0;
        top = atomicAdd(As.wave_done + nm::kTicketTop, 1);
      }
      stage = 2;
    }
  };
  nm::wave_step<real, G, EP>(sh, Ms, As, wave, copy_model, draw);
  if (As.dbg && NM_TID == 0) {
    const unsigned long long t_end = __builtin_amdgcn_s_memtime();
    real* d = As.dbg + (size_t)(wave * G) * nm::kDbgN + 250;
    d[0] = (real)(unsigned)(t_start & 0xFFFFFF); d[1] = (real)(unsigned)((t_start >> 24) & 0xFFFFFF);
    d[2] = (real)(unsigned)(t_end & 0xFFFFFF); d[3] = (real)(unsigned)((t_end >> 24) & 0xFFFFFF);
    d[4] = (real)(__builtin_amdgcn_s_getreg(4 | (0 << 6) | (15 << 11)) & 0xFFFF);
    d[5] = (real)(__builtin_amdgcn_s_getreg(20 | (0 << 6) | (3 << 11)) & 0xF);
  }
  if (As.physics_only) return;
  if (stage < 1) draw(0);
  if (stage < 2) draw(1);
  if (!closes_group) return;
  if (__builtin_amdgcn_readfirstlane(top) != ngrp - 1) return;
#ifndef NM_SKIP_TAIL2
  step_tail<real>(As, Ms.ep_len_s);
#endif
}


template <class real>
__global__ void k_reset(nm::Model<real> M, nm::Args<real> A, const int32_t* ids, int n) {
  int j = blockIdx.x * blockDim.x + threadIdx.x;
  if (j >= n) return;
  int env = ids ? ids[j] : j;
  for (int k = 0; k < nm::kNQ; k++) A.qpos[env * nm::kNQ + k] = M.qpos0[k];
  for (int k = 0; k < nm::kNV; k++) A.qvel[env * nm::kNV + k] = real(0);
  real ux, uy;
  uint32_t ctr = A.rngctr[env];
  if (A.cmd_u) { ux = A.cmd_u[env * 4 + 2]; uy = A.cmd_u[env * 4 + 3]; }
  else {
    ux = (real)nm::rand_u24_bits(A.seed, (uint64_t)(A.env_offset + env), ctr) * real(1.0 / 16777216.0);
    uy = (real)nm::rand_u24_bits(A.seed, (uint64_t)(A.env_offset + env), ctr + 1) * real(1.0 / 16777216.0);
    ctr += 2;
  }
  real c0 = ux * real(2) * M.max_lin_x - M.max_lin_x, c2 = uy * real(2) * M.max_ang - M.max_ang;
  real keep = sqrt(c0 * c0) > real(0.02) ? real(1) : real(0);
  A.cmd[env * 3] = c0 * keep; A.cmd[env * 3 + 1] = real(0); A.cmd[env * 3 + 2] = c2;
  A.rngctr[env] = ctr;
  A.eplen[env] = 0;
  for (int k = 0; k < nm::kNLEG; k++) A.feetair[env * nm::kNLEG + k] = real(0);
  for (int k = 0; k < nm::kNREW; k++) {
    atomicAdd(A.stat_sum + k, A.epsum[env * nm::kNREW + k]);
    A.epsum[env * nm::kNREW + k] = real(0);
  }
  atomicAdd(A.stat_cnt, 1);
}

template <class real>
__global__ void k_finalize(int N, real* stat_sum, int* stat_cnt, float* ep_stats, const float* timeout_now, float* time_outs,
                           real ep_len_s, long long* counters) {
  __shared__ int cnt;
  if (threadIdx.x == 0) cnt = stat_cnt[0];
  __syncthreads();
  if (cnt > 0) {
    if (threadIdx.x < nm::kNREW && ep_stats) ep_stats[threadIdx.x] = (float)(stat_sum[threadIdx.x] / (real)cnt / ep_len_s);
    if (time_outs && timeout_now)
      for (int i = threadIdx.x; i < N; i += blockDim.x) time_outs[i] = timeout_now[i];
  }
  __syncthreads();
  if (threadIdx.x < nm::kNREW) stat_sum[threadIdx.x] = real(0);
  if (threadIdx.x == 0) {
    stat_cnt[0] = 0;
    counters[0] += stat_cnt[1];
    counters[1] += stat_cnt[2];
    counters[2] += stat_cnt[3];
    stat_cnt[1] = 0;
    stat_cnt[2] = 0;
    stat_cnt[3] = 0;
  }
}

template <class real> struct EnvP3 { real v[3]; };
template <class real> struct EnvP3P { const real* p[3]; };
template <class real> struct EnvP3W { real* p[3]; };
template <class real>
__global__ void k_envp_set(real* __restrict__ rows, int N, EnvP3P<real> src, EnvP3<real> dflt) {
  const int i = blockIdx.x * blockDim.x + threadIdx.x;
  if (i >= 4 * N) return;
  const int env = i >> 2, col = i & 3;
  real v = real(0);
  if (col < 3) v = src.p[col] ? src.p[col][env] : dflt.v[col];
  rows[i] = v;
}
template <class real>
__global__ void k_envp_get(const real* __restrict__ rows, int N, EnvP3W<real> dst, EnvP3<real> dflt) {
  const int i = blockIdx.x * blockDim.x + threadIdx.x;
  if (i >= 4 * N) return;
  const int env = i >> 2, col = i & 3;
  if (col < 3 && dst.p[col]) dst.p[col][env] = rows ? rows[i] : dflt.v[col];
}
template <class real> __device__ __forceinline__ real envp_lerp(real lo, real u, real d) {
#pragma clang fp contract(off)
  const real p = u * d;
  return lo + p;
}
template <class real>
__global__ void k_envp_draw(real* __restrict__ rows, int N, uint64_t seed, int64_t env_offset, EnvP3<real> lo, EnvP3<real> hi) {
  const int i = blockIdx.x * blockDim.x + threadIdx.x;
  if (i >= 4 * N) return;
  const int env = i >> 2, col = i & 3;
  real v = real(0);
  if (col < 3) {
    const real u = (real)nm::rand_u24_bits(seed + nm::kEnvParamKey, (uint64_t)(env_offset + env), (uint32_t)col) * real(1.0 / 16777216.0);
    v = envp_lerp(lo.v[col], u, hi.v[col] - lo.v[col]);
  }
  rows[i] = v;
}

template <class real> struct BodyRow { real v[nm::kBodyP]; };
template <class real> struct Pay4 { real v[4]; };
template <class real>
__global__ void k_body_fill(real* __restrict__ rows, int N, BodyRow<real> dflt) {
  const int i = blockIdx.x * blockDim.x + threadIdx.x;
  if (i >= nm::kBodyP * N) return;
  rows[i] = dflt.v[i % nm::kBodyP];
}
template <class real>
__global__ void k_payload_draw(real* __restrict__ out, int N, uint64_t seed, int64_t env_offset, Pay4<real> lo, Pay4<real> hi) {
  const int i = blockIdx.x * blockDim.x + threadIdx.x;
  if (i >= 4 * N) return;
  const int env = i >> 2, col = i & 3;
  const real u = (real)nm::rand_u24_bits(seed + nm::kPayloadKey, (uint64_t)(env_offset + env), (uint32_t)col) * real(1.0 / 16777216.0);
  out[i] = envp_lerp(lo.v[col], u, hi.v[col] - lo.v[col]);
}

__global__ void k_latency_draw(int* __restrict__ delay, int N, uint64_t seed, int64_t env_offset, int lo, int hi) {
  const int e = blockIdx.x * blockDim.x + threadIdx.x;
  if (e >= N) return;
  const uint64_t bits = nm::rand_u24_bits(seed + nm::kLatencyKey, (uint64_t)(env_offset + e), 0u);
  delay[e] = lo + (int)((bits * (uint64_t)(hi - lo + 1)) >> 24);
}

struct nm_env {
  int N = 0, device = 0, dtype = 0;
  virtual ~nm_env() {}
  virtual int reset(const int32_t* ids, int n, int64_t* eplen, float* ep_stats, hipStream_t s) = 0;
  virtual int step(const float* actions, int64_t* eplen, float* obs, float* rew, int64_t* done, float* time_outs, float* ep_stats,
                   int physics_only, hipStream_t s) = 0;
  virtual int get_state(double* qpos, double* qvel, double* qw) = 0;
  virtual int set_state(const double* qpos, const double* qvel, const double* qw) = 0;
  virtual int get_buffers(double* dp, double* dv, double* act, double* cmd, double* es) = 0;
  virtual int set_buffers(const double* dp, const double* dv, const double* act, const double* cmd, const double* es) = 0;
  virtual int set_cmd_u(const double* u) = 0;
  virtual int get_feet(double* air, unsigned char* last, unsigned char* filt) = 0;
  virtual int set_feet(const double* air, const unsigned char* last, const unsigned char* filt) = 0;
  virtual int counters(int64_t* out) = 0;
  virtual void set_dbg(void* p) = 0;
  virtual void set_ret_acc(float* p) = 0;
  virtual int invalidate_time_outs(hipStream_t s) = 0;
  virtual int rollout(const nm_rollout_args* r, int act, hipStream_t s) = 0;
  virtual int rollout_act(const float* flat, const float* obs, uint64_t seed, const int64_t* iter_dev, int step, int act, float* actions, float* logp, float* values,
                          float* mu, float* sigma, float* obs_store, hipStream_t s) = 0;
  virtual int profiling(int on, double* sum_ms, int64_t* count) = 0;
  virtual void set_ablate(int m) = 0;
  virtual int set_noise(const double* vec) = 0;
  virtual int set_noise_u(const double* u) = 0;
  virtual int set_record(int idx) = 0;
  virtual int get_record(double* qpos, double* qvel, int32_t* nbad) = 0;
  virtual int play(const nm_play_args* r, int act, hipStream_t s) = 0;
  virtual int tape(const nm_tape_args* r, hipStream_t s) = 0;
  virtual int get_log(int first, int count, double* rows) = 0;
  virtual int get_log_dones(int first, int count, unsigned char* dones) = 0;
  virtual int set_env_params(const void* mu, const void* p_gain, const void* kv, hipStream_t s) = 0;
  virtual int get_env_params(void* mu, void* p_gain, void* kv, hipStream_t s) = 0;
  virtual int draw_env_params(const double* lo, const double* hi, hipStream_t s) = 0;
  virtual int set_body_params(const void* rows, hipStream_t s) = 0;
  virtual int get_body_params(void* out, hipStream_t s) = 0;
  virtual int draw_payload(const double* lo, const double* hi, void* out, hipStream_t s) = 0;
  virtual int set_action_latency(const int* substeps, hipStream_t s) = 0;
  virtual int get_action_latency(int* out, hipStream_t s) = 0;
  virtual int draw_action_latency(int lo, int hi, hipStream_t s) = 0;
  virtual int set_action_history(const float* h, hipStream_t s) = 0;
  virtual int get_action_history(float* out, hipStream_t s) = 0;
  int push_interval = 0;
  double push_max = 0.0;
  uint64_t push_step = 0;
  int rnoise_on = 0;
  double rnoise_ranges[2 * nm::kResetRanges] = {};
  virtual int set_reset_counts(const uint32_t* counts_host) = 0;
  virtual int get_reset_counts(uint32_t* counts_host) = 0;
};

template <class real> struct Env : nm_env {
  nmhost::Tables<real> T;
  nm::Model<real> M;
  nm::Args<real> A;
  std::vector<void*> allocs;
  real* cmd_u_dev = nullptr;
  bool cmd_u_on = false;
  float* timeout_now = nullptr;
  int32_t* ids_dev = nullptr;
  long long* counters_dev = nullptr;
  nm::Model<real>* M_dev = nullptr;
  real* noise_vec_dev = nullptr;
  real* noise_u_dev = nullptr;
  bool noise_on = false, noise_u_on = false;
  uint64_t noise_step = 0;
  real* rec_dev = nullptr;
  int rec_env = -1;
  real* rec_log = nullptr;
  int rec_log_cap = 0, rec_log_rows = 0;
  unsigned char* rec_done = nullptr;
  bool rec_done_valid = false;
  const real* rec_last = nullptr;
  bool prof_on = false;
  std::vector<std::pair<hipEvent_t, hipEvent_t>> prof_ev;
  size_t prof_used = 0;

  char* slab = nullptr;
  size_t slab_size = 0, slab_used = 0;
  int slab_init(size_t bytes) {
    slab_size = (bytes + (2u << 20) - 1) & ~(size_t)((2u << 20) - 1);
    HIPCHK(hipMalloc((void**)&slab, slab_size));
    HIPCHK(hipMemset(slab, 0, slab_size));
    allocs.push_back(slab);
    return 0;
  }
  template <class X> int dalloc(X** p, size_t n) {
    const size_t bytes = (n * sizeof(X) + 255) & ~(size_t)255;
    if (slab && slab_used + bytes <= slab_size) {
      *p = (X*)(slab + slab_used);
      slab_used += bytes;
      return 0;
    }
    HIPCHK(hipMalloc((void**)p, n * sizeof(X)));
    HIPCHK(hipMemset(*p, 0, n * sizeof(X)));
    allocs.push_back(*p);
    return 0;
  }
  template <class X> int upload(const X** p, const std::vector<X>& v) {
    X* d;
    if (dalloc(&d, v.size())) return 1;
    HIPCHK(hipMemcpy(d, v.data(), v.size() * sizeof(X), hipMemcpyHostToDevice));
    *p = d;
    return 0;
  }
  int init(const nmhost::EnvConfig& cfg, int n, int dev, uint64_t seed, int64_t off) {
    N = n; device = dev; dtype = sizeof(real) == 8;
    HIPCHK(hipSetDevice(dev));
    T.build();
    memset(&M, 0, sizeof M);
    memset(&A, 0, sizeof A);
    T.fill_scalars(M, cfg);
#ifdef NM_MEASURE
    if (const char* e = getenv("NM_MEASURE_PGS_ITERS")) M.pgs_iters = atoi(e);
    if (const char* e = getenv("NM_MEASURE_NOSLIP_ITERS")) M.noslip_iters = atoi(e);
#endif
    if (slab_init((T.hullv.size() + T.hullnv.size()) * sizeof(real) + (size_t)n * 300 * sizeof(real) + (size_t)n * 64 + (1u << 20))) return 1;
    if (upload(&M.hullv, T.hullv) || upload(&M.hullnv, T.hullnv)) return 1;
    A.N = N; A.seed = seed; A.env_offset = off; A.nsub = cfg.decimation;
    {
      int nx = 0;
      if (hipDeviceGetAttribute(&nx, hipDeviceAttributeNumberOfXccs, dev) != hipSuccess) { (void)hipGetLastError(); nx = 0; }
      A.nxcd = nx;
    }
    size_t n_ = (size_t)N;
    if (dalloc(&A.qpos, n_ * 25) || dalloc(&A.qvel, n_ * 24) || dalloc(&A.qwarm, n_ * 24) || dalloc(&A.dofpos, n_ * 18) ||
        dalloc(&A.dofvel, n_ * 18) || dalloc(&A.act, n_ * 18) || dalloc(&A.cmd, n_ * 3) || dalloc(&A.epsum, n_ * nm::kNREW) || dalloc(&A.feetair, n_ * nm::kNLEG) || dalloc(&A.feetflags, n_) ||
        dalloc(&A.rngctr, n_) || dalloc(&A.hullcache, n_ * 8) || dalloc(&A.stat_sum, nm::kNREW) || dalloc(&A.stat_cnt, 4) || dalloc(&cmd_u_dev, n_ * 4) ||
        dalloc(&timeout_now, n_) || dalloc(&ids_dev, n_) || dalloc(&counters_dev, 4) || dalloc(&A.wave_done, ((n_ + nm::kTicketGroup - 1) / nm::kTicketGroup + 2) * nm::kTicketStride) || dalloc(&A.nto, 1) || dalloc(&A.to_list, n_) || dalloc(&A.nprev, 1) || dalloc(&A.to_prev, n_) || dalloc(&A.to_owner, 1))
      return 1;
    if (dalloc(&M_dev, 1)) return 1;
    HIPCHK(hipMemcpy(M_dev, &M, sizeof M, hipMemcpyHostToDevice));
    std::vector<real> q0(n_ * 25);
    for (size_t i = 0; i < n_; i++)
      for (int k = 0; k < 25; k++) q0[i * 25 + k] = T.qpos0[k];
    HIPCHK(hipMemcpy(A.qpos, q0.data(), q0.size() * sizeof(real), hipMemcpyHostToDevice));
    return 0;
  }
  ~Env() override {
    (void)hipSetDevice(device);
    (void)hipDeviceSynchronize();
    for (auto& ev : prof_ev) { (void)hipEventDestroy(ev.first); (void)hipEventDestroy(ev.second); }
    for (void* p : allocs) (void)hipFree(p);
  }
  int finalize(float* ep_stats, float* time_outs, hipStream_t s) {
    hipLaunchKernelGGL(k_finalize<real>, dim3(1), dim3(1024), 0, s, N, A.stat_sum, A.stat_cnt, ep_stats, timeout_now, time_outs, M.ep_len_s,
                       counters_dev);
    HIPCHK(hipGetLastError());
    return 0;
  }
  int reset(const int32_t* ids, int n, int64_t* eplen, float* ep_stats, hipStream_t s) override {
    HIPCHK(hipSetDevice(device));
    if (!eplen) return fail("nm_reset: episode_length_dev is NULL");
    const int32_t* idp = nullptr;
    if (ids) {
      if (n <= 0) return 0;
      for (int i = 0; i < n; i++)
        if (ids[i] < 0 || ids[i] >= N) return fail("nm_reset: env id out of range");
      HIPCHK(hipMemcpyAsync(ids_dev, ids, sizeof(int32_t) * n, hipMemcpyHostToDevice, s));
      HIPCHK(hipStreamSynchronize(s));
      idp = ids_dev;
    } else n = N;
    nm::Args<real> a = A;
    a.eplen = eplen;
    a.cmd_u = cmd_u_on ? cmd_u_dev : nullptr;
    hipLaunchKernelGGL(k_reset<real>, dim3((n + 255) / 256), dim3(256), 0, s, M, a, idp, n);
    HIPCHK(hipGetLastError());
    if (rnoise_on && launch_reset_noise(nullptr, idp, n, s)) return 1;
    return finalize(ep_stats, nullptr, s);
  }
  int step(const float* actions, int64_t* eplen, float* obs, float* rew, int64_t* done, float* time_outs, float* ep_stats, int physics_only,
           hipStream_t s) override {
    HIPCHK(hipSetDevice(device));
    if (!actions) return fail("nm_step: actions_dev is NULL");
    if (!physics_only && (!eplen || !obs || !rew || !done)) return fail("nm_step: NULL output pointer");
    nm::Args<real> a = A;
    a.actions = actions; a.eplen = eplen; a.obs = obs; a.rew = rew; a.done = done; a.timeout_now = timeout_now;
    a.cmd_u = cmd_u_on ? cmd_u_dev : nullptr;
    a.physics_only = physics_only;
    a.ep_stats = ep_stats; a.time_outs = time_outs; a.counters = counters_dev;
    if (!physics_only) {
      a.noise_vec = noise_on ? noise_vec_dev : nullptr;
      a.noise_u = noise_on && noise_u_on ? noise_u_dev : nullptr;
      a.noise_step = noise_step++;
      a.rec = rec_env >= 0 ? rec_dev : nullptr;
      a.rec_env = rec_env;
      if (rec_env >= 0) rec_last = rec_dev;
      const uint64_t ps = push_step++;
      if (nm::push_due(push_interval, ps)) {
        hipLaunchKernelGGL(nm::k_push<real>, dim3((2 * N + 255) / 256), dim3(256), 0, s, A.qvel, N, A.seed, A.env_offset,
                           nm::push_counter(push_interval, ps), (real)push_max);
        HIPCHK(hipGetLastError());
      }
    }
    hipEvent_t e0 = nullptr, e1 = nullptr;
    if (prof_on) {
      if (prof_used == prof_ev.size()) {
        HIPCHK(hipEventCreate(&e0));
        HIPCHK(hipEventCreate(&e1));
        prof_ev.push_back({e0, e1});
      }
      e0 = prof_ev[prof_used].first; e1 = prof_ev[prof_used].second;
      prof_used++;
      HIPCHK(hipEventRecord(e0, s));
    }
    constexpr int G = sizeof(real) == 8 ? 1 : NM_ENVS_PER_WAVE;
    constexpr int W = sizeof(real) == 8 ? 1 : kWG;
    nmrows::with_level(rows.level(physics_only), [&](auto L) {
      hipLaunchKernelGGL((k_env_step<real, G, decltype(L)::value>), dim3((N + G * W - 1) / (G * W)), dim3(64 * W), 0, s, (const nm::Model<real>*)M_dev, a);
    });
    HIPCHK(hipGetLastError());
    if (prof_on) HIPCHK(hipEventRecord(e1, s));
    if (!physics_only && rnoise_on && launch_reset_noise(done, nullptr, N, s)) return 1;
    return 0;
  }
  int d2h(const real* dev, double* host, size_t n) {
    if (!host) return 0;
    std::vector<real> tmp(n);
    HIPCHK(hipMemcpy(tmp.data(), dev, n * sizeof(real), hipMemcpyDeviceToHost));
    for (size_t i = 0; i < n; i++) host[i] = (double)tmp[i];
    return 0;
  }
  int h2d(real* dev, const double* host, size_t n) {
    if (!host) return 0;
    std::vector<real> tmp(n);
    for (size_t i = 0; i < n; i++) tmp[i] = (real)host[i];
    HIPCHK(hipMemcpy(dev, tmp.data(), n * sizeof(real), hipMemcpyHostToDevice));
    return 0;
  }
  int get_state(double* qpos, double* qvel, double* qw) override {
    HIPCHK(hipSetDevice(device));
    HIPCHK(hipDeviceSynchronize());
    return d2h(A.qpos, qpos, (size_t)N * 25) || d2h(A.qvel, qvel, (size_t)N * 24) || d2h(A.qwarm, qw, (size_t)N * 24);
  }
  int set_state(const double* qpos, const double* qvel, const double* qw) override {
    HIPCHK(hipSetDevice(device));
    HIPCHK(hipDeviceSynchronize());
    return h2d(A.qpos, qpos, (size_t)N * 25) || h2d(A.qvel, qvel, (size_t)N * 24) || h2d(A.qwarm, qw, (size_t)N * 24);
  }
  int get_buffers(double* dp, double* dv, double* act, double* cmd, double* es) override {
    HIPCHK(hipSetDevice(device));
    HIPCHK(hipDeviceSynchronize());
    return d2h(A.dofpos, dp, (size_t)N * 18) || d2h(A.dofvel, dv, (size_t)N * 18) || d2h(A.act, act, (size_t)N * 18) ||
           d2h(A.cmd, cmd, (size_t)N * 3) || d2h(A.epsum, es, (size_t)N * nm::kNREW);
  }
  int set_buffers(const double* dp, const double* dv, const double* act, const double* cmd, const double* es) override {
    HIPCHK(hipSetDevice(device));
    HIPCHK(hipDeviceSynchronize());
    return h2d(A.dofpos, dp, (size_t)N * 18) || h2d(A.dofvel, dv, (size_t)N * 18) || h2d(A.act, act, (size_t)N * 18) ||
           h2d(A.cmd, cmd, (size_t)N * 3) || h2d(A.epsum, es, (size_t)N * nm::kNREW);
  }
  int get_feet(double* air, unsigned char* last, unsigned char* filt) override {
    HIPCHK(hipSetDevice(device));
    HIPCHK(hipDeviceSynchronize());
    if (d2h(A.feetair, air, (size_t)N * 6)) return 1;
    std::vector<int> fl(N);
    HIPCHK(hipMemcpy(fl.data(), A.feetflags, sizeof(int) * N, hipMemcpyDeviceToHost));
    for (int i = 0; i < N; i++)
      for (int k = 0; k < 6; k++) {
        if (last) last[i * 6 + k] = (fl[i] >> k) & 1;
        if (filt) filt[i * 6 + k] = (fl[i] >> (6 + k)) & 1;
      }
    return 0;
  }
  int set_feet(const double* air, const unsigned char* last, const unsigned char* filt) override {
    HIPCHK(hipSetDevice(device));
    HIPCHK(hipDeviceSynchronize());
    if (h2d(A.feetair, air, (size_t)N * 6)) return 1;
    if (last || filt) {
      std::vector<int> fl(N);
      HIPCHK(hipMemcpy(fl.data(), A.feetflags, sizeof(int) * N, hipMemcpyDeviceToHost));
      for (int i = 0; i < N; i++)
        for (int k = 0; k < 6; k++) {
          if (last) fl[i] = (fl[i] & ~(1 << k)) | ((last[i * 6 + k] ? 1 : 0) << k);
          if (filt) fl[i] = (fl[i] & ~(1 << (6 + k))) | ((filt[i * 6 + k] ? 1 : 0) << (6 + k));
        }
      HIPCHK(hipMemcpy(A.feetflags, fl.data(), sizeof(int) * N, hipMemcpyHostToDevice));
    }
    return 0;
  }
  int set_cmd_u(const double* u) override {
    HIPCHK(hipSetDevice(device));
    HIPCHK(hipDeviceSynchronize());
    cmd_u_on = u != nullptr;
    return h2d(cmd_u_dev, u, (size_t)N * 4);
  }
  int counters(int64_t* out) override {
    HIPCHK(hipSetDevice(device));
    HIPCHK(hipDeviceSynchronize());
    long long c[3];
    HIPCHK(hipMemcpy(c, counters_dev, sizeof c, hipMemcpyDeviceToHost));
    std::vector<int> hc((size_t)N * 8);
    HIPCHK(hipMemcpy(hc.data(), A.hullcache, hc.size() * sizeof(int), hipMemcpyDeviceToHost));
    long long fb = 0;
    for (int i = 0; i < N; i++) fb += hc[(size_t)i * 8 + 7];
    out[0] = c[0]; out[1] = c[1]; out[2] = fb;
    return 0;
  }
  int set_noise(const double* vec) override {
    HIPCHK(hipSetDevice(device));
    HIPCHK(hipDeviceSynchronize());
    noise_on = vec != nullptr;
    if (vec && !noise_vec_dev && dalloc(&noise_vec_dev, NM_NUM_OBS)) return 1;
    return vec ? h2d(noise_vec_dev, vec, NM_NUM_OBS) : 0;
  }
  int set_noise_u(const double* u) override {
    HIPCHK(hipSetDevice(device));
    HIPCHK(hipDeviceSynchronize());
    noise_u_on = u != nullptr;
    if (u && !noise_u_dev && dalloc(&noise_u_dev, (size_t)N * NM_NUM_OBS)) return 1;
    return u ? h2d(noise_u_dev, u, (size_t)N * NM_NUM_OBS) : 0;
  }
  int set_record(int idx) override {
    HIPCHK(hipSetDevice(device));
    HIPCHK(hipDeviceSynchronize());
    if (idx >= N) return fail("nm_set_state_record: env index out of range");
    if (idx >= 0 && !rec_dev && dalloc(&rec_dev, 64)) return 1;
    rec_env = idx < 0 ? -1 : idx;
    rec_last = nullptr; rec_log_rows = 0; rec_done_valid = false;
    return 0;
  }
  int get_record(double* qpos, double* qvel, int32_t* nbad) override {
    HIPCHK(hipSetDevice(device));
    if (rec_env < 0) return fail("nm_get_state_record: recording is off (nm_set_state_record)");
    if (!rec_last) return fail("nm_get_state_record: no step has been recorded yet");
    HIPCHK(hipDeviceSynchronize());
    double tmp[50];
    if (d2h(rec_last, tmp, 50)) return 1;
    if (qpos) for (int i = 0; i < 25; i++) qpos[i] = tmp[i];
    if (qvel) for (int i = 0; i < 24; i++) qvel[i] = tmp[25 + i];
    if (nbad) *nbad = (int32_t)tmp[49];
    return 0;
  }

  int get_log(int first, int count, double* rows) override {
    HIPCHK(hipSetDevice(device));
    if (rec_env < 0) return fail("nm_get_state_log: recording is off (nm_set_state_record)");
    if (first < 0 || count < 0 || first + count > rec_log_rows) return fail("nm_get_state_log: rows outside the last K-step launch");
    if (count == 0) return 0;
    if (!rows) return fail("nm_get_state_log: rows_host is NULL");
    HIPCHK(hipDeviceSynchronize());
    return d2h(rec_log + (size_t)first * nmr::kRecRow, rows, (size_t)count * nmr::kRecRow);
  }
  int get_log_dones(int first, int count, unsigned char* dones) override {
    HIPCHK(hipSetDevice(device));
    if (rec_env < 0) return fail("nm_get_state_log_dones: recording is off (nm_set_state_record)");
    if (!rec_done_valid) return fail("nm_get_state_log_dones: the last K-step launch was not nm_play (nm_rollout files the flags in its dones rows)");
    if (first < 0 || count < 0 || first + count > rec_log_rows) return fail("nm_get_state_log_dones: steps outside the last K-step launch");
    if (count == 0) return 0;
    if (!dones) return fail("nm_get_state_log_dones: dones_host is NULL");
    HIPCHK(hipDeviceSynchronize());
    HIPCHK(hipMemcpy(dones, rec_done + first, (size_t)count, hipMemcpyDeviceToHost));
    return 0;
  }
  int log_rows(int K, real** out) {
    *out = nullptr;
    if (rec_env < 0) return 0;
    if (K > rec_log_cap) {
      if (dalloc(&rec_log, (size_t)roll_cap * nmr::kRecRow) || dalloc(&rec_done, (size_t)roll_cap)) return 1;
      rec_log_cap = roll_cap;
    }
    rec_log_rows = K;
    rec_done_valid = false;
    rec_last = rec_log + (size_t)(K - 1) * nmr::kRecRow;
    *out = rec_log;
    return 0;
  }
  int roll_reserve(int K) {
    if (K > roll_cap) {
      const int cap = (K + 127) & ~127;
      if (dalloc(&roll_sum, (size_t)cap * nm::kNREW) || dalloc(&roll_cnt, (size_t)cap * 4)) return 1;
      if (!roll_to && dalloc(&roll_to, (size_t)N)) return 1;
      roll_cap = cap;
    }
    return 0;
  }
  float *roll_wp = nullptr, *roll_bp = nullptr;
  real* roll_sum = nullptr;
  int *roll_cnt = nullptr, *roll_to = nullptr;
  int roll_cap = 0;
  typedef nmr::RefShape RS;
  int roll_pack(const float* flat, hipStream_t s) {
    if (!roll_wp && (dalloc(&roll_wp, (size_t)RS::nfrag() * 256) || dalloc(&roll_bp, (size_t)RS::nbias()))) return 1;
    if (nmr::launch_pack(flat, roll_wp, roll_bp, s)) return fail("nm_rollout: packing the policy failed to launch");
    return 0;
  }
  int rollout_act(const float* flat, const float* obs, uint64_t seed, const int64_t* iter_dev, int step, int act, float* actions, float* logp, float* values,
                  float* mu, float* sigma, float* obs_store, hipStream_t s) override {
    HIPCHK(hipSetDevice(device));
    if (!flat || !obs || !iter_dev || !actions || !logp || !values || !mu || !sigma) return fail("nm_rollout_act: NULL pointer");
    if (roll_pack(flat, s)) return 1;
    nmr::ActOut o{actions, logp, values, mu, sigma, obs_store};
    if (nmr::launch_act(roll_wp, roll_bp, flat + RS::stdoff(), obs, N, seed, iter_dev, step, o, act, s)) return fail("nm_rollout_act: launch failed");
    return 0;
  }
  int kstep_check(const char* who, int K, const char* hint, int n_ep, const int* ep_idx, const float* ep_acc, const float* ep_stats) {
    if (K < 1 || K > 4096) return fail(std::string(who) + ": steps must be in 1..4096" + hint);
    if (n_ep < 0 || n_ep > nm::kNREW || (n_ep > 0 && (!ep_idx || !ep_acc || !ep_stats))) return fail(std::string(who) + ": bad episode-statistics arguments");
    return 0;
  }
  nm::Args<real> kstep_args(int K, const float* actions, int64_t* eplen, float* obs, float* rew, int64_t* done, real* log) {
    nm::Args<real> a = A;
    a.actions = actions; a.eplen = eplen; a.obs = obs; a.rew = rew; a.done = done; a.timeout_now = timeout_now;
    a.cmd_u = cmd_u_on ? cmd_u_dev : nullptr;
    a.physics_only = 0;
    a.ep_stats = nullptr; a.time_outs = nullptr; a.counters = counters_dev;
    a.to_list = nullptr;
    a.noise_vec = noise_on ? noise_vec_dev : nullptr;
    a.noise_u = noise_on && noise_u_on ? noise_u_dev : nullptr;
    a.noise_step = noise_step;
    noise_step += (uint64_t)K;
    a.rec = log; a.rec_env = log ? rec_env : -1; a.dbg = nullptr; a.ret_acc = nullptr;
    return a;
  }
  uint32_t* rnoise_count = nullptr;
  int rnoise_reserve() {
    if (rnoise_count) return 0;
    if (dalloc(&rnoise_count, (size_t)N)) return 1;
    HIPCHK(hipMemset(rnoise_count, 0, (size_t)N * sizeof(uint32_t)));
    HIPCHK(hipDeviceSynchronize());
    return 0;
  }
  int set_reset_counts(const uint32_t* counts_host) override {
    HIPCHK(hipSetDevice(device));
    if (rnoise_reserve()) return 1;
    if (!counts_host) return 0;
    HIPCHK(hipDeviceSynchronize());
    HIPCHK(hipMemcpy(rnoise_count, counts_host, (size_t)N * sizeof(uint32_t), hipMemcpyHostToDevice));
    return 0;
  }
  int get_reset_counts(uint32_t* counts_host) override {
    if (!counts_host) return 0;
    if (!rnoise_count) { memset(counts_host, 0, (size_t)N * sizeof(uint32_t)); return 0; }
    HIPCHK(hipSetDevice(device));
// ... 557 lines not shown
```

### nightmare_rl_amd/csrc/simt.h

```cpp
#pragma once
#include <stdint.h>

#define NM_WAVE 64

#ifndef NM_EMUL
#include <hip/hip_runtime.h>
#define NM_FN __device__ __forceinline__
#define NM_HDFN __host__ __device__ __forceinline__
#define NM_COLD __device__ __noinline__
namespace simt {
template <class T> using V = T;
using VB = bool;

#ifdef NM_WG_WAVES
#define NM_TID ((int)(threadIdx.x & 63))
#else
#define NM_TID ((int)threadIdx.x)
#endif
NM_FN int lane_id() { return NM_TID; }
template <class T> NM_FN T sel(bool c, T a, T b) { return c ? a : b; }
NM_FN float vsqrt(float x) { return sqrtf(x); }
NM_FN double vsqrt(double x) { return sqrt(x); }
NM_FN float vabs(float x) { return fabsf(x); }
NM_FN double vabs(double x) { return fabs(x); }
NM_FN float vmax(float a, float b) { return fmaxf(a, b); }
NM_FN double vmax(double a, double b) { return fmax(a, b); }
NM_FN float vmin(float a, float b) { return fminf(a, b); }
NM_FN double vmin(double a, double b) { return fmin(a, b); }
NM_FN int vmin(int a, int b) { return a < b ? a : b; }
NM_FN int vmax(int a, int b) { return a > b ? a : b; }
NM_FN void vsincos(float x0, float* s, float* c) {
  const float x = fminf(fmaxf(x0, -4194304.0f), 4194304.0f);
  const float k = rintf(x * 0.636619772f);
  float r = fmaf(-k, 1.5707963705062866f, x);
  r = fmaf(-k, -4.371139000186241e-8f, r);
  const float r2 = r * r;
  const float ps = fmaf(r * r2, fmaf(r2, fmaf(r2, -1.9515295891e-4f, 8.3321608736e-3f), -1.6666654611e-1f), r);
  const float pc = fmaf(r2 * r2, fmaf(r2, fmaf(r2, 2.443315711809948e-5f, -1.388731625493765e-3f), 4.166664568298827e-2f), fmaf(r2, -0.5f, 1.0f));
  const int n = (int)k;
  const float sa = (n & 1) ? pc : ps, ca = (n & 1) ? ps : pc;
  *s = (n & 2) ? -sa : sa;
  *c = ((n + 1) & 2) ? -ca : ca;
}
NM_FN void vsincos(double x, double* s, double* c) { sincos(x, s, c); }
NM_FN float vexp(float x) { return expf(x); }
NM_FN double vexp(double x) { return exp(x); }
NM_FN float vacos(float x) { return acosf(x); }
NM_FN double vacos(double x) { return acos(x); }
NM_FN float vpow(float x, float p) { return powf(x, p); }
NM_FN double vpow(double x, double p) { return pow(x, p); }
NM_FN bool visbad(float x) { return !(fabsf(x) <= 1e10f); }
NM_FN bool visbad(double x) { return !(fabs(x) <= 1e10); }
template <class T> NM_FN T to_real(int i) { return (T)i; }
template <class T, class S> NM_FN T vcvt(S x) { return (T)x; }
NM_FN float vrcp(float x) { return __builtin_amdgcn_rcpf(x); }
NM_FN double vrcp(double x) { return 1.0 / x; }

NM_FN float vfma(float a, float b, float c) { return __builtin_fmaf(a, b, c); }
NM_FN double vfma(double a, double b, double c) { return __builtin_fma(a, b, c); }
NM_FN float sel_mask(uint64_t m, float a, float b) {
  float r;
  asm("v_cndmask_b32_e64 %0, %1, %2, %3" : "=v"(r) : "v"(b), "v"(a), "s"(m));
  return r;
}
NM_FN double sel_mask(uint64_t m, double a, double b) {
  int rl, rh;
  asm("v_cndmask_b32_e64 %0, %2, %3, %6\n\tv_cndmask_b32_e64 %1, %4, %5, %6" : "=&v"(rl), "=v"(rh)
      : "v"(__double2loint(b)), "v"(__double2loint(a)), "v"(__double2hiint(b)), "v"(__double2hiint(a)), "s"(m));
  return __hiloint2double(rh, rl);
}
NM_FN uint64_t mask_shl(uint64_t m, int k) { m <<= k; asm("" : "+s"(m)); return m; }
template <int I> NM_FN float fma_half_lane(float a, float x, float g, bool h1);
template <int I> NM_FN double fma_half_lane(double a, double x, double g, bool h1);
NM_FN int rdlane(int x, int l) { return __builtin_amdgcn_readlane(x, l); }
NM_FN float rdlane(float x, int l) { return __int_as_float(__builtin_amdgcn_readlane(__float_as_int(x), l)); }
NM_FN double rdlane(double x, int l) {
  int lo = __builtin_amdgcn_readlane(__double2loint(x), l), hi = __builtin_amdgcn_readlane(__double2hiint(x), l);
  return __hiloint2double(hi, lo);
}
template <int I> NM_FN float fma_half_lane(float a, float x, float g, bool h1) {
  const float s0 = rdlane(x, I), s1 = rdlane(x, 32 + I);
  return vfma(a, h1 ? s1 : s0, g);
}
template <int I> NM_FN double fma_half_lane(double a, double x, double g, bool h1) {
  const double s0 = rdlane(x, I), s1 = rdlane(x, 32 + I);
  return vfma(a, h1 ? s1 : s0, g);
}
template <class T> NM_FN T wrlane(T x, T v, int l) {
  int ln = NM_TID;
  asm volatile("" : "+v"(ln));
  return ln == l ? v : x;
}
NM_FN int opaque_lane() { int ln = NM_TID; asm volatile("" : "+v"(ln)); return ln; }
template <class T> NM_FN T uniform(T x) { return rdlane(x, 0); }
NM_FN bool uniform(bool x) { return __builtin_amdgcn_readfirstlane((int)x) != 0; }
#define NM_DPP_QUAD_XOR1 0xB1
#define NM_DPP_QUAD_XOR2 0x4E
#define NM_DPP_HALF_MIRROR 0x141
#define NM_DPP_ROW_MIRROR 0x140
template <int CTRL> NM_FN int dpp(int x) { return __builtin_amdgcn_mov_dpp(x, CTRL, 0xF, 0xF, true); }
template <int CTRL> NM_FN float dpp(float x) { return __int_as_float(dpp<CTRL>(__float_as_int(x))); }
template <int CTRL> NM_FN double dpp(double x) { return __hiloint2double(dpp<CTRL>(__double2hiint(x)), dpp<CTRL>(__double2loint(x))); }
template <int P, class T> NM_FN T quad(T x) { return dpp<P>(x); }
template <class T> NM_FN T shfl_xor1(T x) { return dpp<NM_DPP_QUAD_XOR1>(x); }
template <class T> NM_FN T shfl_xor2(T x) { return dpp<NM_DPP_QUAD_XOR2>(x); }
template <class T> NM_FN T wsum8(T x) {
  x = x + dpp<NM_DPP_QUAD_XOR1>(x);
  x = x + dpp<NM_DPP_QUAD_XOR2>(x);
  x = x + dpp<NM_DPP_HALF_MIRROR>(x);
  return rdlane(x, 0);
}
template <class T> NM_FN T gsum8(T x) {
  x = x + dpp<NM_DPP_QUAD_XOR1>(x);
  x = x + dpp<NM_DPP_QUAD_XOR2>(x);
  x = x + dpp<NM_DPP_HALF_MIRROR>(x);
  return x;
}
template <class T> NM_FN T wsum(T x) {
  x = x + dpp<NM_DPP_QUAD_XOR1>(x);
  x = x + dpp<NM_DPP_QUAD_XOR2>(x);
  x = x + dpp<NM_DPP_HALF_MIRROR>(x);
  x = x + dpp<NM_DPP_ROW_MIRROR>(x);
  return (rdlane(x, 0) + rdlane(x, 16)) + (rdlane(x, 32) + rdlane(x, 48));
}
template <class T> NM_FN T hsum32(T x) {
  x = x + dpp<NM_DPP_QUAD_XOR1>(x);
  x = x + dpp<NM_DPP_QUAD_XOR2>(x);
  x = x + dpp<NM_DPP_HALF_MIRROR>(x);
  x = x + dpp<NM_DPP_ROW_MIRROR>(x);
  const T s0 = rdlane(x, 0) + rdlane(x, 16), s1 = rdlane(x, 32) + rdlane(x, 48);
  return (NM_TID & 32) ? s1 : s0;
}
NM_FN bool wany(bool c) { return __ballot(c) != 0ull; }
NM_FN int lane_rank(uint64_t m) { return (int)__builtin_amdgcn_mbcnt_hi((uint32_t)(m >> 32), __builtin_amdgcn_mbcnt_lo((uint32_t)m, 0u)); }
NM_FN int popc64(uint64_t m) { return __popcll(m); }
NM_FN uint64_t ballot(bool c) { return __ballot(c); }
NM_FN bool in_mask(uint64_t m) { return __builtin_amdgcn_inverse_ballot_w64(m); }
template <class T> NM_FN void order_after(int& a, const T& dep) { asm volatile("" : "+v"(a) : "v"(dep)); }
template <class T> NM_FN void wargmax(T val, int idx, T* best, int* ibest) {
#define NM_AM_STEP(CTRL)                                                   \
  {                                                                        \
    T ov = dpp<CTRL>(val);                                                 \
    int oi = dpp<CTRL>(idx);                                               \
    bool take = (ov > val) | ((ov == val) & (oi < idx));                   \
    val = take ? ov : val;                                                 \
    idx = take ? oi : idx;                                                 \
  }
  NM_AM_STEP(NM_DPP_QUAD_XOR1) NM_AM_STEP(NM_DPP_QUAD_XOR2) NM_AM_STEP(NM_DPP_HALF_MIRROR) NM_AM_STEP(NM_DPP_ROW_MIRROR)
#undef NM_AM_STEP
  T bv = rdlane(val, 0);
  int bi = rdlane(idx, 0);
#pragma unroll
  for (int r = 16; r < 64; r += 16) {
    T ov = rdlane(val, r);
    int oi = rdlane(idx, r);
    bool take = (ov > bv) | ((ov == bv) & (oi < bi));
    bv = take ? ov : bv;
    bi = take ? oi : bi;
  }
  *best = bv;
  *ibest = bi;
}
template <class T> NM_FN void wmaxfirst(T val, T* best, int* lane_of_best) {
  T m = val;
  m = vmax(m, dpp<NM_DPP_QUAD_XOR1>(m));
  m = vmax(m, dpp<NM_DPP_QUAD_XOR2>(m));
  m = vmax(m, dpp<NM_DPP_HALF_MIRROR>(m));
  m = vmax(m, dpp<NM_DPP_ROW_MIRROR>(m));
  const T b = vmax(vmax(rdlane(m, 0), rdlane(m, 16)), vmax(rdlane(m, 32), rdlane(m, 48)));
  *best = b;
  *lane_of_best = (int)__builtin_ctzll(__ballot(val == b));
}
template <class T> NM_FN T ldsv(const T* a, int i) { return a[i]; }
template <class T> NM_FN void stsv(T* a, int i, T v, bool m) { if (m) a[i] = v; }
template <class T, class S> NM_FN void stsu(T* a, int i, T v, bool m, S* sink) {
  T* p = m ? a + i : reinterpret_cast<T*>(sink) + NM_TID;
  *p = v;
}
#define NM_GLOBAL(T) __attribute__((address_space(1))) T
typedef float nm_f4 __attribute__((ext_vector_type(4)));
typedef double nm_d4 __attribute__((ext_vector_type(4)));
template <class T> NM_FN T gldv(const T* p, int i) { return ((const NM_GLOBAL(T)*)p)[i]; }
template <class T> NM_FN void gstv(T* p, int i, T v, bool m) { if (m) ((NM_GLOBAL(T)*)p)[i] = v; }
template <class T> NM_FN T gld1(const T* p, size_t i) { return ((const NM_GLOBAL(T)*)p)[i]; }
template <class T> NM_FN void gst1(T* p, size_t i, T v) { ((NM_GLOBAL(T)*)p)[i] = v; }
NM_FN void gadd1(float* p, size_t i, float v) { __builtin_amdgcn_global_atomic_fadd_f32((NM_GLOBAL(float)*)p + i, v); }
NM_FN void gld3(const float* p, int i, float* o) { const nm_f4 t = *(const NM_GLOBAL(nm_f4)*)((const NM_GLOBAL(float)*)p + i); o[0] = t.x; o[1] = t.y; o[2] = t.z; }
NM_FN void gld3(const double* p, int i, double* o) { const nm_d4 t = *(const NM_GLOBAL(nm_d4)*)((const NM_GLOBAL(double)*)p + i); o[0] = t.x; o[1] = t.y; o[2] = t.z; }
NM_FN void gld4(const float* p, int i, float* o) { const nm_f4 t = *(const NM_GLOBAL(nm_f4)*)((const NM_GLOBAL(float)*)p + i); o[0] = t.x; o[1] = t.y; o[2] = t.z; o[3] = t.w; }
NM_FN void gld4(const double* p, int i, double* o) { const nm_d4 t = *(const NM_GLOBAL(nm_d4)*)((const NM_GLOBAL(double)*)p + i); o[0] = t.x; o[1] = t.y; o[2] = t.z; o[3] = t.w; }
NM_FN int to_int(float x) { return (int)x; }
NM_FN int to_int(double x) { return (int)x; }
NM_FN void wave_sync() {
  __builtin_amdgcn_fence(__ATOMIC_RELEASE, "wavefront");
  __builtin_amdgcn_wave_barrier();
  __builtin_amdgcn_fence(__ATOMIC_ACQUIRE, "wavefront");
}
NM_FN void sched_fence() { __builtin_amdgcn_sched_barrier(0); }
}

#else
#include <cmath>
#include <cstring>
#define NM_FN inline
#define NM_HDFN inline
#define NM_COLD inline
namespace simt {
template <class T> struct V {
  T v[NM_WAVE];
  V() {}
  V(T s) { for (int i = 0; i < NM_WAVE; i++) v[i] = s; }
#define NM_BIN(op)                                                                                   \
  friend V operator op(const V& a, const V& b) { V r; for (int i = 0; i < NM_WAVE; i++) r.v[i] = a.v[i] op b.v[i]; return r; }
  NM_BIN(+) NM_BIN(-) NM_BIN(*) NM_BIN(/) NM_BIN(%) NM_BIN(&) NM_BIN(|) NM_BIN(>>) NM_BIN(<<)
#undef NM_BIN
#define NM_CMP(op)                                                                                      \
  friend V<bool> operator op(const V& a, const V& b) { V<bool> r; for (int i = 0; i < NM_WAVE; i++) r.v[i] = a.v[i] op b.v[i]; return r; }
  NM_CMP(<) NM_CMP(>) NM_CMP(<=) NM_CMP(>=) NM_CMP(==) NM_CMP(!=)
#undef NM_CMP
  friend V operator-(const V& a) { V r; for (int i = 0; i < NM_WAVE; i++) r.v[i] = -a.v[i]; return r; }
  friend V operator!(const V& a) { V r; for (int i = 0; i < NM_WAVE; i++) r.v[i] = !a.v[i]; return r; }
  V& operator+=(const V& b) { for (int i = 0; i < NM_WAVE; i++) v[i] += b.v[i]; return *this; }
  V& operator-=(const V& b) { for (int i = 0; i < NM_WAVE; i++) v[i] -= b.v[i]; return *this; }
  V& operator*=(const V& b) { for (int i = 0; i < NM_WAVE; i++) v[i] *= b.v[i]; return *this; }
};
using VB = V<bool>;

NM_FN V<int> lane_id() { V<int> r; for (int i = 0; i < NM_WAVE; i++) r.v[i] = i; return r; }
#define NM_SEL(T)                                                                                              \
  NM_FN V<T> sel(const VB& c, const V<T>& a, const V<T>& b) { V<T> r; for (int i = 0; i < NM_WAVE; i++) r.v[i] = c.v[i] ? a.v[i] : b.v[i]; return r; } \
  NM_FN T sel(bool c, T a, T b) { return c ? a : b; }
NM_SEL(float) NM_SEL(double) NM_SEL(int)
#undef NM_SEL
#define NM_MAP1(name, expr)                                                                                   \
  NM_FN V<float> name(const V<float>& a) { V<float> r; for (int i = 0; i < NM_WAVE; i++) { float x = a.v[i]; r.v[i] = expr; } return r; } \
  NM_FN V<double> name(const V<double>& a) { V<double> r; for (int i = 0; i < NM_WAVE; i++) { double x = a.v[i]; r.v[i] = expr; } return r; } \
  NM_FN float name(float x) { return expr; }                                                                  \
  NM_FN double name(double x) { return expr; }
NM_MAP1(vsqrt, std::sqrt(x)) NM_MAP1(vabs, std::fabs(x)) NM_MAP1(vexp, std::exp(x)) NM_MAP1(vacos, std::acos(x))
#undef NM_MAP1
#define NM_MAP2(name, expr, T)                                                                               \
  NM_FN V<T> name(const V<T>& a, const V<T>& b) { V<T> r; for (int i = 0; i < NM_WAVE; i++) { T x = a.v[i], y = b.v[i]; r.v[i] = expr; } return r; } \
  NM_FN T name(T x, T y) { return expr; }
NM_MAP2(vmax, (x > y ? x : y), float) NM_MAP2(vmax, (x > y ? x : y), double) NM_MAP2(vmax, (x > y ? x : y), int)
NM_MAP2(vmin, (x < y ? x : y), float) NM_MAP2(vmin, (x < y ? x : y), double) NM_MAP2(vmin, (x < y ? x : y), int)
NM_MAP2(vpow, std::pow(x, y), float) NM_MAP2(vpow, std::pow(x, y), double)
#undef NM_MAP2
template <class T> NM_FN void vsincos(const V<T>& x, V<T>* s, V<T>* c) { for (int i = 0; i < NM_WAVE; i++) { s->v[i] = std::sin(x.v[i]); c->v[i] = std::cos(x.v[i]); } }
NM_FN void vsincos(float x, float* s, float* c) { *s = std::sin(x); *c = std::cos(x); }
NM_FN void vsincos(double x, double* s, double* c) { *s = std::sin(x); *c = std::cos(x); }
template <class T> NM_FN VB visbad(const V<T>& a) { VB r; for (int i = 0; i < NM_WAVE; i++) r.v[i] = !(std::fabs(a.v[i]) <= (T)1e10); return r; }
NM_FN bool visbad(float x) { return !(std::fabs(x) <= 1e10f); }
NM_FN bool visbad(double x) { return !(std::fabs(x) <= 1e10); }
template <class T> NM_FN V<T> to_real(const V<int>& a) { V<T> r; for (int i = 0; i < NM_WAVE; i++) r.v[i] = (T)a.v[i]; return r; }
template <class T> NM_FN T to_real(int a) { return (T)a; }
template <class T> NM_FN V<T> vrcp(const V<T>& a) { V<T> r; for (int i = 0; i < NM_WAVE; i++) r.v[i] = (T)1 / a.v[i]; return r; }
NM_FN float vrcp(float x) { return 1.0f / x; }
NM_FN double vrcp(double x) { return 1.0 / x; }
template <class T, class S> NM_FN V<T> vcvt(const V<S>& a) { V<T> r; for (int i = 0; i < NM_WAVE; i++) r.v[i] = (T)a.v[i]; return r; }

template <class T> NM_FN V<T> vfma(const V<T>& a, const V<T>& b, const V<T>& c) { return a * b + c; }
NM_FN float vfma(float a, float b, float c) { return a * b + c; }
NM_FN double vfma(double a, double b, double c) { return a * b + c; }
template <class T> NM_FN V<T> sel_mask(uint64_t m, const V<T>& a, const V<T>& b) {
  V<T> r;
  for (int i = 0; i < NM_WAVE; i++) r.v[i] = ((m >> i) & 1ull) ? a.v[i] : b.v[i];
  return r;
}
NM_FN uint64_t mask_shl(uint64_t m, int k) { return m << k; }
template <int I, class T> NM_FN V<T> fma_half_lane(const V<T>& a, const V<T>& x, const V<T>& g, const VB&) {
  V<T> r;
  for (int i = 0; i < NM_WAVE; i++) r.v[i] = a.v[i] * x.v[(i & 32) + I] + g.v[i];
  return r;
}
template <class T> NM_FN T rdlane(const V<T>& x, int l) { return x.v[l]; }
template <class T> NM_FN T rdlane(T x, int) { return x; }
template <class T> NM_FN V<T> wrlane(V<T> x, T v, int l) { x.v[l] = v; return x; }
NM_FN V<int> opaque_lane() { return lane_id(); }
template <class T> NM_FN T uniform(const V<T>& x) { return x.v[0]; }
template <class T> NM_FN T uniform(T x) { return x; }
template <class T> NM_FN V<T> shfl_xor(const V<T>& x, int m) { V<T> r; for (int i = 0; i < NM_WAVE; i++) r.v[i] = x.v[i ^ m]; return r; }
template <int P, class T> NM_FN V<T> quad(const V<T>& x) { V<T> r; for (int i = 0; i < NM_WAVE; i++) r.v[i] = x.v[(i & ~3) | ((P >> (2 * (i & 3))) & 3)]; return r; }
template <class T> NM_FN V<T> shfl_xor1(const V<T>& x) { return shfl_xor(x, 1); }
template <class T> NM_FN V<T> shfl_xor2(const V<T>& x) { return shfl_xor(x, 2); }
template <class T> NM_FN V<T> half_mirror(const V<T>& x) { V<T> r; for (int i = 0; i < NM_WAVE; i++) r.v[i] = x.v[(i & ~7) | (7 - (i & 7))]; return r; }
template <class T> NM_FN V<T> row_mirror(const V<T>& x) { V<T> r; for (int i = 0; i < NM_WAVE; i++) r.v[i] = x.v[(i & ~15) | (15 - (i & 15))]; return r; }
template <class T> NM_FN V<T> gsum8(V<T> x) {
  x = x + shfl_xor(x, 1); x = x + shfl_xor(x, 2); x = x + half_mirror(x);
  return x;
}
template <class T> NM_FN T wsum8(V<T> x) {
  x = x + shfl_xor(x, 1); x = x + shfl_xor(x, 2); x = x + half_mirror(x);
  return x.v[0];
}
template <class T> NM_FN T wsum(V<T> x) {
  x = x + shfl_xor(x, 1); x = x + shfl_xor(x, 2); x = x + half_mirror(x); x = x + row_mirror(x);
  return (x.v[0] + x.v[16]) + (x.v[32] + x.v[48]);
}
template <class T> NM_FN V<T> hsum32(V<T> x) {
  x = x + shfl_xor(x, 1); x = x + shfl_xor(x, 2); x = x + half_mirror(x); x = x + row_mirror(x);
  const T s0 = x.v[0] + x.v[16], s1 = x.v[32] + x.v[48];
  V<T> r; for (int i = 0; i < NM_WAVE; i++) r.v[i] = i < 32 ? s0 : s1;
  return r;
}
NM_FN bool wany(const VB& c) { for (int i = 0; i < NM_WAVE; i++) if (c.v[i]) return true; return false; }
NM_FN V<int> lane_rank(uint64_t m) { V<int> r; for (int i = 0; i < NM_WAVE; i++) r.v[i] = __builtin_popcountll(m & ((1ull << i) - 1ull)); return r; }
NM_FN int popc64(uint64_t m) { return __builtin_popcountll(m); }
NM_FN uint64_t ballot(const VB& c) { uint64_t m = 0; for (int i = 0; i < NM_WAVE; i++) if (c.v[i]) m |= 1ull << i; return m; }
NM_FN VB in_mask(uint64_t m) { VB r; for (int i = 0; i < NM_WAVE; i++) r.v[i] = (m >> i) & 1; return r; }
template <class T> NM_FN void order_after(V<int>&, const V<T>&) {}
template <class T> NM_FN void wargmax(V<T> val, V<int> idx, T* best, int* ibest) {
  T bv = val.v[0]; int bi = idx.v[0];
  for (int i = 1; i < NM_WAVE; i++)
    if (val.v[i] > bv || (val.v[i] == bv && idx.v[i] < bi)) { bv = val.v[i]; bi = idx.v[i]; }
  *best = bv; *ibest = bi;
}
template <class T> NM_FN void wmaxfirst(const V<T>& val, T* best, int* lane_of_best) {
  T bv = val.v[0]; int bi = 0;
  for (int i = 1; i < NM_WAVE; i++) if (val.v[i] > bv) { bv = val.v[i]; bi = i; }
  *best = bv; *lane_of_best = bi;
}
template <class T> NM_FN V<T> ldsv(const T* a, const V<int>& i) { V<T> r; for (int k = 0; k < NM_WAVE; k++) r.v[k] = a[i.v[k]]; return r; }
template <class T> NM_FN T ldsv(const T* a, int i) { return a[i]; }
template <class T> NM_FN void stsv(T* a, const V<int>& i, const V<T>& v, const VB& m) { for (int k = 0; k < NM_WAVE; k++) if (m.v[k]) a[i.v[k]] = v.v[k]; }
template <class T> NM_FN void stsv(T* a, const V<int>& i, T v, const VB& m) { for (int k = 0; k < NM_WAVE; k++) if (m.v[k]) a[i.v[k]] = v; }
template <class T, class S> NM_FN void stsu(T* a, const V<int>& i, const V<T>& v, const VB& m, S*) { stsv(a, i, v, m); }
template <class T, class S> NM_FN void stsu(T* a, const V<int>& i, T v, const VB& m, S*) { stsv(a, i, v, m); }
template <class T> NM_FN T gld1(const T* p, size_t i) { return p[i]; }
template <class T> NM_FN void gst1(T* p, size_t i, T v) { p[i] = v; }
NM_FN void gadd1(float* p, size_t i, float v) { p[i] += v; }
template <class T> NM_FN V<T> gldv(const T* p, const V<int>& i) { return ldsv(p, i); }
template <class T> NM_FN void gstv(T* p, const V<int>& i, const V<T>& v, const VB& m) { stsv(p, i, v, m); }
template <class T> NM_FN void gstv(T* p, const V<int>& i, T v, const VB& m) { stsv(p, i, v, m); }
template <class T> NM_FN void gld4(const T* p, const V<int>& i, V<T>* o) { for (int k = 0; k < NM_WAVE; k++) for (int c = 0; c < 4; c++) o[c].v[k] = p[i.v[k] + c]; }
template <class T> NM_FN V<int> to_int(const V<T>& a) { V<int> r; for (int i = 0; i < NM_WAVE; i++) r.v[i] = (int)a.v[i]; return r; }
template <class T> NM_FN void gld3(const T* p, const V<int>& i, V<T>* o) { for (int k = 0; k < NM_WAVE; k++) for (int c = 0; c < 3; c++) o[c].v[k] = p[i.v[k] + c]; }
template <class T> NM_FN void gld3(const T* p, int i, T* o) { o[0] = p[i]; o[1] = p[i + 1]; o[2] = p[i + 2]; }
NM_FN void wave_sync() {}
NM_FN void sched_fence() {}
}
#endif
```

Before: 83.76 million env-steps/s.

## Read launch args from kernarg segment and vectorize model copy to LDS

```diff
diff --git a/nightmare_rl_amd/csrc/nm_core.h b/nightmare_rl_amd/csrc/nm_core.h
--- a/nightmare_rl_amd/csrc/nm_core.h
+++ b/nightmare_rl_amd/csrc/nm_core.h
@@ -51,6 +51,15 @@
   int collide_batch_min;
   real tibia_max, body_max, base_h_target, max_contact_force;
 };
+
+constexpr size_t kModelRound = 64 * 16;
+template <class real> union alignas(16) ModelBlock {
+  Model<real> m;
+  unsigned char bytes[(sizeof(Model<real>) + kModelRound - 1) / kModelRound * kModelRound];
+};
+static_assert(sizeof(ModelBlock<float>) % kModelRound == 0 && sizeof(ModelBlock<double>) % kModelRound == 0 &&
+              sizeof(ModelBlock<float>) - sizeof(Model<float>) < kModelRound && sizeof(ModelBlock<double>) - sizeof(Model<double>) < kModelRound,
+              "ModelBlock: whole copy rounds, less than one round of padding");
 
 template <class real> struct Args {
   int N;
@@ -102,6 +111,34 @@
 template <class real> NM_FN float* lat_hist(const Args<real>& A) { return reinterpret_cast<float*>(lat_delay(A) + A.N); }
 constexpr int kDbgN = 256;
 
+template <class Src> struct ArgSrc { static constexpr bool kScalarBase = false; };
+template <class real> NM_FN const Args<real>& launch_args(const Args<real>& a) { return a; }
+template <class real> NM_FN const Args<real>& launch_args(const Args<real>* a) { return *a; }
+#ifndef NM_EMUL
+typedef const __attribute__((address_space(4))) char* kernarg_ptr;
+template <class real, int OFS> struct KernArgs { kernarg_ptr seg; };
+template <class real, int OFS> struct ArgSrc<KernArgs<real, OFS>> { static constexpr bool kScalarBase = true; };
+template <class real, int OFS> NM_FN const Args<real>& launch_args(const KernArgs<real, OFS>& k) {
+  kernarg_ptr p = k.seg;
+  asm volatile("" : "+s"(p));
+  return *(const Args<real>*)(const __attribute__((address_space(4))) Args<real>*)(p + OFS);
+}
+template <class real, int OFS> NM_FN void launch_args_touch(const KernArgs<real, OFS>& k) {
+  kernarg_ptr p = k.seg;
+  asm volatile("" : "+s"(p));
+  int x = 0;
+#pragma unroll
+  for (int o = 0; o < OFS + (int)sizeof(Args<real>); o += 64) x |= *(const __attribute__((address_space(4))) int*)(p + o);
+  asm volatile("" ::"s"(x));
+}
+template <class real> NM_FN const Args<real>* scalar_src(const Args<real>* a) { return a; }
+template <class real, int OFS> NM_FN KernArgs<real, OFS> scalar_src(const KernArgs<real, OFS>& k) {
+  const uint64_t u = (uint64_t)k.seg;
+  const uint32_t lo = (uint32_t)__builtin_amdgcn_readfirstlane((int)(uint32_t)u), hi = (uint32_t)__builtin_amdgcn_readfirstlane((int)(uint32_t)(u >> 32));
+  return KernArgs<real, OFS>{(kernarg_ptr)(((uint64_t)hi << 32) | lo)};
+}
+#endif
+
 template <class real> struct Sh {
   real qpos[kNQ];
   real envp[kEnvPS];
@@ -3014,8 +3051,10 @@
 }
 
 struct NoMid { NM_FN void operator()() const {} NM_FN void operator()(int) const {} };
-template <int EP, class real, class Mid> NM_FN void env_load2(ShW<real, 2>& w, const Model<real>& M, const Args<real>& A, int wave, Mid&& mid) {
+template <int EP, class real, class Src, class Mid> NM_FN void env_load2(ShW<real, 2>& w, const Model<real>& M, const Src& src, int wave, Mid&& mid) {
   typedef V<real> vr;
+  const Args<real>& A = launch_args(src);
+  constexpr bool kS = ArgSrc<Src>::kScalarBase;
   constexpr int kSR = (int)(sizeof(Sh<real>) / sizeof(real)), kSI = (int)(sizeof(Sh<real>) / sizeof(int));
   const V<int> lane = opaque_lane();
   const V<int> h = lane >> 5, hl = lane & 31;
@@ -3026,39 +3065,39 @@
   const V<int> ho = h * kSR, hoi = h * kSI;
   const VB l18 = hl < kNU;
   const V<int> l18c = sel(l18, hl, V<int>(0));
-  const vr q_in = gldv(A.qpos, sel(hl < kNQ, hl, V<int>(0)) + env * kNQ);
-  const vr v_in = gldv(A.qvel, sel(hl < kNV, hl, V<int>(0)) + env * kNV);
-  const vr w_in = gldv(A.qwarm, sel(hl < kNV, hl, V<int>(0)) + env * kNV);
-  const V<int> hc_in = gldv(A.hullcache, sel(hl < 8, hl, V<int>(0)) + env * 8);
-  const V<float> a_in = gldv(A.actions, l18c + env * kNU);
+  const vr q_in = gldx<kS>(A.qpos, sel(hl < kNQ, hl, V<int>(0)) + env * kNQ);
+  const vr v_in = gldx<kS>(A.qvel, sel(hl < kNV, hl, V<int>(0)) + env * kNV);
+  const vr w_in = gldx<kS>(A.qwarm, sel(hl < kNV, hl, V<int>(0)) + env * kNV);
+  const V<int> hc_in = gldx<kS>(A.hullcache, sel(hl < 8, hl, V<int>(0)) + env * 8);
+  const V<float> a_in = gldx<kS>(A.actions, l18c + env * kNU);
   vr envp_in = vr(real(0));
-  if constexpr (EP != 0) envp_in = gldv(A.envp, sel(hl < kEnvP, hl, V<int>(0)) + env * kEnvP);
+  if constexpr (EP != 0) envp_in = gldx<kS>(A.envp, sel(hl < kEnvP, hl, V<int>(0)) + env * kEnvP);
   vr body_in = vr(real(0));
-  if constexpr (EP >= 2) body_in = gldv(A.envp, sel(hl < kBodyP, hl, V<int>(0)) + (env * kBodyP + A.N * kEnvP));
+  if constexpr (EP >= 2) body_in = gldx<kS>(A.envp, sel(hl < kBodyP, hl, V<int>(0)) + (env * kBodyP + A.N * kEnvP));
   vr cmd_in = vr(real(0)), eps_in = vr(real(0)), prev_act = vr(real(0)), prev_dofvel = vr(real(0)), dofpos_old = vr(real(0));
   V<int> dl = V<int>(0);
   V<float> h0 = V<float>(0.0f), h1 = V<float>(0.0f), h2 = V<float>(0.0f);
   if constexpr (EP == 3)
     if (!A.physics_only) {
-      dl = gldv(lat_delay(A), env);
-      h0 = gldv(lat_hist(A), l18c + env * (kLatH * kNU));
-      h1 = gldv(lat_hist(A), l18c + (env * (kLatH * kNU) + kNU));
-      h2 = gldv(lat_hist(A), l18c + (env * (kLatH * kNU) + 2 * kNU));
+      dl = gldx<kS>(lat_delay(A), env);
+      h0 = gldx<kS>(lat_hist(A), l18c + env * (kLatH * kNU));
+      h1 = gldx<kS>(lat_hist(A), l18c + (env * (kLatH * kNU) + kNU));
+      h2 = gldx<kS>(lat_hist(A), l18c + (env * (kLatH * kNU) + 2 * kNU));
     }
 #ifndef NM_EMUL
   int64_t ep = 0;
   uint32_t ctr_in = 0;
 #endif
   if (!A.physics_only) {
-    cmd_in = gldv(A.cmd, sel(hl < 3, hl, V<int>(0)) + env * 3);
-    eps_in = gldv(A.epsum, sel(hl < kNREW, hl, V<int>(0)) + env * kNREW);
+    cmd_in = gldx<kS>(A.cmd, sel(hl < 3, hl, V<int>(0)) + env * 3);
+    eps_in = gldx<kS>(A.epsum, sel(hl < kNREW, hl, V<int>(0)) + env * kNREW);
 #ifndef NM_EMUL
-    ep = gld1(A.eplen, (size_t)env);
-    ctr_in = gld1(A.rngctr, (size_t)env);
+    ep = gld1x<kS>(A.eplen, env);
+    ctr_in = gld1x<kS>(A.rngctr, env);
 #endif
-    prev_act = gldv(A.act, l18c + env * kNU);
-    prev_dofvel = gldv(A.dofvel, l18c + env * kNU);
-    dofpos_old = gldv(A.dofpos, l18c + env * kNU);
+    prev_act = gldx<kS>(A.act, l18c + env * kNU);
+    prev_dofvel = gldx<kS>(A.dofvel, l18c + env * kNU);
+    dofpos_old = gldx<kS>(A.dofpos, l18c + env * kNU);
   }
   mid();
   stsv(rb, ho + (hl + NM_OFS(qpos)), q_in, hl < kNQ);
@@ -3115,9 +3154,9 @@
       stsv(L.rsw, h, r, hl == zero);
       float* hist = lat_hist(A);
       const VB st = l18 & (env0 < V<int>(A.N));
-      gstv(hist, hl + (env * (kLatH * kNU) + 2 * kNU), h1, st);
-      gstv(hist, hl + (env * (kLatH * kNU) + kNU), h0, st);
-      gstv(hist, hl + env * (kLatH * kNU), af, st);
+      gstx<kS>(hist, hl + (env * (kLatH * kNU) + 2 * kNU), h1, st);
+      gstx<kS>(hist, hl + (env * (kLatH * kNU) + kNU), h0, st);
+      gstx<kS>(hist, hl + env * (kLatH * kNU), af, st);
     } else
     stsv(rb, ho + (hl + NM_OFS(ctrl)), ((act - defp) - dofpos_old) * p_gain, l18);
   } else {
@@ -3129,8 +3168,10 @@
   wave_sync();
 }
 
-template <class real, class Pub> NM_FN void env_finish2(ShW<real, 2>& w, const Model<real>& M, const Args<real>& A, int wave, int dropped, Pub&& published) {
+template <class real, class Src, class Pub> NM_FN void env_finish2(ShW<real, 2>& w, const Model<real>& M, const Src& src, int wave, int dropped, Pub&& published) {
   typedef V<real> vr;
+  const Args<real>& A = launch_args(src);
+  constexpr bool kS = ArgSrc<Src>::kScalarBase;
   constexpr int kSR = (int)(sizeof(Sh<real>) / sizeof(real)), kSI = (int)(sizeof(Sh<real>) / sizeof(int));
   const V<int> lane = opaque_lane();
   const V<int> h = lane >> 5, hl = lane & 31;
@@ -3157,15 +3198,15 @@
     V<int> hc = SHI(hcache, sel(hl < 8, hl, V<int>(0)));
     hc = sel(hl == 0, hc | (SHI(ncon, V<int>(0)) << 16), hc);
     const vr q = SHR(qpos, sel(hl < kNQ, hl, V<int>(0))), v = SHR(qvel, sel(hl < kNV, hl, V<int>(0))), wq = SHR(warm, sel(hl < kNV, hl, V<int>(0)));
-    gstv(A.hullcache, hl + env * 8, hc, live & (hl < 8));
-    gstv(A.qpos, hl + env * kNQ, q, live & (hl < kNQ));
-    gstv(A.qvel, hl + env * kNV, v, live & (hl < kNV));
-    gstv(A.qwarm, hl + env * kNV, wq, live & (hl < kNV));
+    gstx<kS>(A.hullcache, hl + env * 8, hc, live & (hl < 8));
+    gstx<kS>(A.qpos, hl + env * kNQ, q, live & (hl < kNQ));
+    gstx<kS>(A.qvel, hl + env * kNV, v, live & (hl < kNV));
+    gstx<kS>(A.qwarm, hl + env * kNV, wq, live & (hl < kNV));
     if (A.rec) {
       const VB r = live & (env == V<int>(A.rec_env));
-      gstv(A.rec, hl, q, r & (hl < kNQ));
-      gstv(A.rec, hl + kNQ, v, r & (hl < kNV));
-      gstv(A.rec, V<int>(kNQ + kNV), to_real<real>(nwarn), r & (hl == 0));
+      gstx<kS>(A.rec, hl, q, r & (hl < kNQ));
+      gstx<kS>(A.rec, hl + kNQ, v, r & (hl < kNV));
+      gstx<kS>(A.rec, V<int>(kNQ + kNV), to_real<real>(nwarn), r & (hl == 0));
     }
   }
   if (A.dbg) {
@@ -3264,8 +3305,8 @@
   const VB resetL = reset & live;
   const uint64_t rmask = ballot(resetL);
   if (rmask) {
-    gstv(A.qpos, hl + env * kNQ, ldsv(M.qpos0, sel(hl < kNQ, hl, V<int>(0))), resetL & (hl < kNQ));
-    gstv(A.qvel, hl + env * kNV, real(0), resetL & (hl < kNV));
+    gstx<kS>(A.qpos, hl + env * kNQ, ldsv(M.qpos0, sel(hl < kNQ, hl, V<int>(0))), resetL & (hl < kNQ));
+    gstx<kS>(A.qvel, hl + env * kNV, real(0), resetL & (hl < kNV));
 #pragma unroll
     for (int hh = 0; hh < 2; hh++)
       if ((rmask >> (32 * hh)) & 1) { resample(hh, 1); ep[hh] = 0; }
@@ -3322,8 +3363,8 @@
       vr over = sel(ff > vr(M.max_contact_force), ff - M.max_contact_force, vr(real(0)));
       rt[R_FEET_CONTACT] = hsum32(sel(l6, over * over, vr(real(0)))) * M.rew_scale[R_FEET_CONTACT];
       if (M.rew_scale[R_FEET_AIR_TIME] != real(0)) {
-        vr air = gldv(A.feetair, l6c + envc * kNLEG);
-        const V<int> fl = gldv(A.feetflags, envc);
+        vr air = gldx<kS>(A.feetair, l6c + envc * kNLEG);
+        const V<int> fl = gldx<kS>(A.feetflags, envc);
         air = sel(reset, vr(real(0)), air);
         const VB contact = ff > vr(real(1));
         const VB filt = contact | (((fl >> l6c) & 1) != 0);
@@ -3332,10 +3373,10 @@
         air = sel(filt == lastf, air, vr(real(0)));
         const vr single = sel(air > vr(real(1)), air - real(1), vr(real(0))) + sel(air < vr(real(0.5)), real(0.5) - air, vr(real(0)));
         rt[R_FEET_AIR_TIME] = hsum32(sel(l6, single * single, vr(real(0)))) * M.rew_scale[R_FEET_AIR_TIME];
-        gstv(A.feetair, l6c + env * kNLEG, air, live & l6);
+        gstx<kS>(A.feetair, l6c + env * kNLEG, air, live & l6);
         const uint64_t bc = ballot(l6 & contact), bf = ballot(l6 & filt);
         const int nf0 = (int)((bc & 63) | ((bf & 63) << kNLEG)), nf1 = (int)(((bc >> 32) & 63) | (((bf >> 32) & 63) << kNLEG));
-        gstv(A.feetflags, env, sel(h1, V<int>(nf1), V<int>(nf0)), live & (hl == 0));
+        gstx<kS>(A.feetflags, env, sel(h1, V<int>(nf1), V<int>(nf0)), live & (hl == 0));
       }
     }
   }
@@ -3346,7 +3387,7 @@
     vr add = vr(real(0));
 #pragma unroll
     for (int k = 0; k < kNREW; k++) add = sel(hl == k, rt[k], add);
-    gstv(A.epsum, hl + env * kNREW, epsum + add, live & (hl < kNREW));
+    gstx<kS>(A.epsum, hl + env * kNREW, epsum + add, live & (hl < kNREW));
   }
   published(1);
   NM_ESTAMP(14);
@@ -3375,7 +3416,8 @@
 #ifdef NM_EMUL
       for (int i = 0; i < NM_WAVE; i++) if (m.v[i]) A.obs[(size_t)env.v[i] * kNOBS + idx.v[i]] = (float)cx.v[i];
 #else
-      if (m) gst1(A.obs, (size_t)env * kNOBS + idx, (float)cx);
+      if constexpr (kS) { if (m) gst1x<true>(A.obs, env * kNOBS + idx, (float)cx); }
+      else if (m) gst1(A.obs, (size_t)env * kNOBS + idx, (float)cx);
 #endif
     };
     put(o, hl, hl < 12);
@@ -3384,12 +3426,12 @@
     put(act, hl + 48, l18);
   }
   NM_ESTAMP(15);
-  gstv(A.dofpos, hl + env * kNU, dofpos, live & l18);
-  gstv(A.dofvel, hl + env * kNU, dofvel, live & l18);
-  gstv(A.act, hl + env * kNU, act, live & l18);
+  gstx<kS>(A.dofpos, hl + env * kNU, dofpos, live & l18);
+  gstx<kS>(A.dofvel, hl + env * kNU, dofvel, live & l18);
+  gstx<kS>(A.act, hl + env * kNU, act, live & l18);
   {
     vr cv = sel(hl == 0, cmd[0], sel(hl == 1, cmd[1], cmd[2]));
-    gstv(A.cmd, hl + env * 3, cv, live & (hl < 3));
+    gstx<kS>(A.cmd, hl + env * 3, cv, live & (hl < 3));
   }
 #ifdef NM_EMUL
   for (int hh = 0; hh < 2; hh++)
@@ -3401,12 +3443,12 @@
     }
 #else
   if (hl == 0 && live) {
-    gst1(A.eplen, (size_t)env, h1 ? ep[1] : ep[0]);
-    gst1(A.rngctr, (size_t)env, h1 ? ctr[1] : ctr[0]);
-    gst1(A.rew, (size_t)env, (float)rew);
-    if (A.ret_acc) gadd1(A.ret_acc, (size_t)env, (float)rew);
-    gst1(A.done, (size_t)env, (int64_t)(reset ? 1 : 0));
-    gst1(A.timeout_now, (size_t)env, time_out ? 1.0f : 0.0f);
+    gst1x<kS>(A.eplen, env, h1 ? ep[1] : ep[0]);
+    gst1x<kS>(A.rngctr, env, h1 ? ctr[1] : ctr[0]);
+    gst1x<kS>(A.rew, env, (float)rew);
+    if (A.ret_acc) gadd1x<kS>(A.ret_acc, env, (float)rew);
+    gst1x<kS>(A.done, env, (int64_t)(reset ? 1 : 0));
+    gst1x<kS>(A.timeout_now, env, time_out ? 1.0f : 0.0f);
   }
 #endif
 #undef SHR
@@ -3431,11 +3473,12 @@
   wave_sync();
 }
 
-template <class real, int G, int EP = 0, class Mid = NoMid, class Pub = NoMid>
-NM_FN void wave_step(ShW<real, G>& w, const Model<real>& M, const Args<real>& A, int wave, Mid&& mid = Mid(), Pub&& published = Pub()) {
+template <class real, int G, int EP = 0, class Mid = NoMid, class Pub = NoMid, class Src = Args<real>>
+NM_FN void wave_step(ShW<real, G>& w, const Model<real>& M, const Src& src, int wave, Mid&& mid = Mid(), Pub&& published = Pub()) {
+  const Args<real>& A = launch_args(src);
   nm_stamp(-1);
   if constexpr (G == 2) {
-    env_load2<EP>(w, M, A, wave, mid);
+    env_load2<EP>(w, M, src, wave, mid);
   } else {
     mid();
 #pragma unroll
@@ -3457,7 +3500,7 @@
     substep<EP>(w, M, s == A.nsub - 1, &dropped, NM_ABLATE(A.ablate));
   }
   if constexpr (G == 2) {
-    env_finish2(w, M, A, wave, dropped, published);
+    env_finish2(w, M, src, wave, dropped, published);
   } else {
 #pragma unroll
     for (int e = 0; e < G; e++) {
diff --git a/nightmare_rl_amd/csrc/nm_hip.hip b/nightmare_rl_amd/csrc/nm_hip.hip
--- a/nightmare_rl_amd/csrc/nm_hip.hip
+++ b/nightmare_rl_amd/csrc/nm_hip.hip
@@ -29,7 +29,8 @@
 #ifndef NM_ENVS_PER_WAVE
 #define NM_ENVS_PER_WAVE 2
 #endif
-template <class real> __device__ __noinline__ void step_tail(const nm::Args<real>& A, real ep_len_s) {
+template <class real, class Src> __device__ __noinline__ void step_tail(Src src, real ep_len_s) {
+  const nm::Args<real>& A = nm::launch_args(nm::scalar_src(src));
   const int lane = NM_TID;
 #define TAIL_LD(p) __hip_atomic_load(p, __ATOMIC_RELAXED, __HIP_MEMORY_SCOPE_AGENT)
   const int cnt = TAIL_LD(A.stat_cnt);
@@ -76,37 +77,51 @@
 #else
 constexpr int kWG = 1;
 #endif
+struct NoArgsCopy {};
+template <class real> __device__ __forceinline__ nm::KernArgs<real, 8> step_src(NoArgsCopy&) { return {(nm::kernarg_ptr)__builtin_amdgcn_kernarg_segment_ptr()}; }
+template <class real> __device__ __forceinline__ const nm::Args<real>& step_src(nm::Args<real>& a) { return a; }
 template <class real, int G, int EP>
 __global__ void __launch_bounds__(64 * (sizeof(real) == 8 ? 1 : kWG), NM_WAVES_PER_SIMD) k_env_step(const nm::Model<real>* __restrict__ Mp, nm::Args<real> A) {
   constexpr int kWG = sizeof(real) == 8 ? 1 : ::kWG;
+  static_assert(sizeof(Mp) == 8 && alignof(nm::Args<real>) == 8, "k_env_step: Args starts at byte 8 of the kernarg segment");
   __shared__ typename nm::ShWSel<real, G, EP>::type shs[kWG];
-  __shared__ nm::Model<real> Ms;
-  __shared__ nm::Args<real> As;
+  __shared__ nm::ModelBlock<real> Mb;
+  const nm::Model<real>& Ms = Mb.m;
+  constexpr bool kKern = sizeof(real) == 4;
+  __shared__ std::conditional_t<kKern, NoArgsCopy, nm::Args<real>> As;
+  decltype(auto) KA = step_src<real>(As);
   nm::ShW<real, G>& sh = nm::ShWSel<real, G, EP>::images(shs[kWG == 1 ? 0 : (int)(threadIdx.x >> 6)]);
-  int wave = nmr::wave_index(A.nxcd);
-  if (kWG > 1) wave = wave * kWG + (int)(threadIdx.x >> 6);
+  if constexpr (kKern) nm::launch_args_touch(KA);
+  else { As = A; __syncthreads(); }
+  int wave;
+  unsigned long long t_start = 0ull;
+  {
+    const nm::Args<real>& A0 = nm::launch_args(KA);
+    const int N = A0.N, nxcd = A0.nxcd;
+    const bool dbg_on = A0.dbg != nullptr;
 #ifdef NM_MEASURE
-  if (A.ablate & 512) return;
+    if (A0.ablate & 512) return;
 #endif
-  const unsigned long long t_start = A.dbg ? __builtin_amdgcn_s_memtime() : 0ull;
-  if (kWG == 1 || threadIdx.x < 64) As = A;
-  __syncthreads();
-  if (wave * G >= A.N) return;
+    wave = nmr::wave_index(nxcd);
+    if (kWG > 1) wave = wave * kWG + (int)(threadIdx.x >> 6);
+    if (dbg_on) t_start = __builtin_amdgcn_s_memtime();
+    if (wave * G >= N) return;
+  }
   auto copy_model = [&]() {
-    const uint32_t* src = reinterpret_cast<const uint32_t*>(Mp);
-    uint32_t* dst = reinterpret_cast<uint32_t*>(&Ms);
-    constexpr int kWords = (int)(sizeof(nm::Model<real>) / 4);
-    uint32_t tmp[(kWords + 63) / 64];
+    typedef uint32_t u4 __attribute__((ext_vector_type(4)));
+    constexpr int kRounds = (int)(sizeof(nm::ModelBlock<real>) / (64 * 16));
+    const NM_GLOBAL(u4)* src = (const NM_GLOBAL(u4)*)Mp;
+    u4* dst = reinterpret_cast<u4*>(&Mb);
+    u4 tmp[kRounds];
 #pragma unroll
-    for (int k = 0; k < (kWords + 63) / 64; k++) { const int i = NM_TID + 64 * k; tmp[k] = i < kWords ? src[i] : 0u; }
+    for (int k = 0; k < kRounds; k++) tmp[k] = src[NM_TID + 64 * k];
     if (kWG == 1 || threadIdx.x < 64) {
 #pragma unroll
-      for (int k = 0; k < (kWords + 63) / 64; k++) { const int i = NM_TID + 64 * k; if (i < kWords) dst[i] = tmp[k]; }
-    }
-    __syncthreads();
+      for (int k = 0; k < kRounds; k++) dst[NM_TID + 64 * k] = tmp[k];
+    }
+    if (kWG == 1) nm::wave_sync(); else __syncthreads();
   };
-  const int nw = (As.N + G - 1) / G, grp = wave / nm::kTicketGroup, ngrp = (nw + nm::kTicketGroup - 1) / nm::kTicketGroup;
-  const int gsize = min(nm::kTicketGroup, nw - grp * nm::kTicketGroup);
+  const int grp = wave / nm::kTicketGroup;
   int ticket = 0, top = 0;
   int stage = 0;
   bool closes_group = false;
@@ -114,34 +129,40 @@
 #ifdef NM_NO_TICKETS
     stage = 2; (void)phase; return;
 #endif
+    const nm::Args<real>& Ad = nm::launch_args(KA);
+    int* wave_done = Ad.wave_done;
     if (phase == 0) {
-      if (NM_TID == 0) ticket = atomicAdd(As.wave_done + (grp + 1) * nm::kTicketStride, 1);
+      if (NM_TID == 0) ticket = atomicAdd(wave_done + (grp + 1) * nm::kTicketStride, 1);
       stage = 1;
     } else {
+      const int nw = (Ad.N + G - 1) / G, gsize = min(nm::kTicketGroup, nw - grp * nm::kTicketGroup);
       closes_group = __builtin_amdgcn_readfirstlane(ticket) == gsize - 1;
       if (closes_group && NM_TID == 0) {
-        As.wave_done[(grp + 1) * nm::kTicketStride] = 0;
-        top = atomicAdd(As.wave_done + nm::kTicketTop, 1);
+        wave_done[(grp + 1) * nm::kTicketStride] = 0;
+        top = atomicAdd(wave_done + nm::kTicketTop, 1);
       }
       stage = 2;
     }
   };
-  nm::wave_step<real, G, EP>(sh, Ms, As, wave, copy_model, draw);
-  if (As.dbg && NM_TID == 0) {
+  nm::wave_step<real, G, EP>(sh, Ms, KA, wave, copy_model, draw);
+  const nm::Args<real>& A1 = nm::launch_args(KA);
+  if (A1.dbg && NM_TID == 0) {
     const unsigned long long t_end = __builtin_amdgcn_s_memtime();
-    real* d = As.dbg + (size_t)(wave * G) * nm::kDbgN + 250;
+    real* d = A1.dbg + (size_t)(wave * G) * nm::kDbgN + 250;
     d[0] = (real)(unsigned)(t_start & 0xFFFFFF); d[1] = (real)(unsigned)((t_start >> 24) & 0xFFFFFF);
     d[2] = (real)(unsigned)(t_end & 0xFFFFFF); d[3] = (real)(unsigned)((t_end >> 24) & 0xFFFFFF);
     d[4] = (real)(__builtin_amdgcn_s_getreg(4 | (0 << 6) | (15 << 11)) & 0xFFFF);
     d[5] = (real)(__builtin_amdgcn_s_getreg(20 | (0 << 6) | (3 << 11)) & 0xF);
   }
-  if (As.physics_only) return;
+  if (A1.physics_only) return;
   if (stage < 1) draw(0);
   if (stage < 2) draw(1);
   if (!closes_group) return;
+  const int ngrp = ((A1.N + G - 1) / G + nm::kTicketGroup - 1) / nm::kTicketGroup;
   if (__builtin_amdgcn_readfirstlane(top) != ngrp - 1) return;
 #ifndef NM_SKIP_TAIL2
-  step_tail<real>(As, Ms.ep_len_s);
+  if constexpr (kKern) step_tail<real>(KA, Ms.ep_len_s);
+  else step_tail<real>(&As, Ms.ep_len_s);
 #endif
 }
 
@@ -388,7 +409,11 @@
         dalloc(&A.rngctr, n_) || dalloc(&A.hullcache, n_ * 8) || dalloc(&A.stat_sum, nm::kNREW) || dalloc(&A.stat_cnt, 4) || dalloc(&cmd_u_dev, n_ * 4) ||
         dalloc(&timeout_now, n_) || dalloc(&ids_dev, n_) || dalloc(&counters_dev, 4) || dalloc(&A.wave_done, ((n_ + nm::kTicketGroup - 1) / nm::kTicketGroup + 2) * nm::kTicketStride) || dalloc(&A.nto, 1) || dalloc(&A.to_list, n_) || dalloc(&A.nprev, 1) || dalloc(&A.to_prev, n_) || dalloc(&A.to_owner, 1))
       return 1;
-    if (dalloc(&M_dev, 1)) return 1;
+    {
+      nm::ModelBlock<real>* mb = nullptr;
+      if (dalloc(&mb, 1)) return 1;
+      M_dev = &mb->m;
+    }
     HIPCHK(hipMemcpy(M_dev, &M, sizeof M, hipMemcpyHostToDevice));
     std::vector<real> q0(n_ * 25);
     for (size_t i = 0; i < n_; i++)
diff --git a/nightmare_rl_amd/csrc/simt.h b/nightmare_rl_amd/csrc/simt.h
--- a/nightmare_rl_amd/csrc/simt.h
+++ b/nightmare_rl_amd/csrc/simt.h
@@ -185,6 +185,18 @@
 template <class T> NM_FN T gld1(const T* p, size_t i) { return ((const NM_GLOBAL(T)*)p)[i]; }
 template <class T> NM_FN void gst1(T* p, size_t i, T v) { ((NM_GLOBAL(T)*)p)[i] = v; }
 NM_FN void gadd1(float* p, size_t i, float v) { __builtin_amdgcn_global_atomic_fadd_f32((NM_GLOBAL(float)*)p + i, v); }
+template <class T> NM_FN const NM_GLOBAL(T)* gofs(const T* p, int i) {
+  return (const NM_GLOBAL(T)*)((const NM_GLOBAL(char)*)p + (uint32_t)i * (uint32_t)sizeof(T));
+}
+template <bool S, class T> NM_FN T gldx(const T* p, int i) { if constexpr (S) return *gofs(p, i); else return gldv(p, i); }
+template <bool S, class T> NM_FN void gstx(T* p, int i, T v, bool m) {
+  if constexpr (S) { if (m) *(NM_GLOBAL(T)*)gofs(p, i) = v; } else gstv(p, i, v, m);
+}
+template <bool S, class T> NM_FN T gld1x(const T* p, int i) { if constexpr (S) return *gofs(p, i); else return gld1(p, (size_t)i); }
+template <bool S, class T> NM_FN void gst1x(T* p, int i, T v) { if constexpr (S) *(NM_GLOBAL(T)*)gofs(p, i) = v; else gst1(p, (size_t)i, v); }
+template <bool S> NM_FN void gadd1x(float* p, int i, float v) {
+  if constexpr (S) __builtin_amdgcn_global_atomic_fadd_f32((NM_GLOBAL(float)*)gofs(p, i), v); else gadd1(p, (size_t)i, v);
+}
 NM_FN void gld3(const float* p, int i, float* o) { const nm_f4 t = *(const NM_GLOBAL(nm_f4)*)((const NM_GLOBAL(float)*)p + i); o[0] = t.x; o[1] = t.y; o[2] = t.z; }
 NM_FN void gld3(const double* p, int i, double* o) { const nm_d4 t = *(const NM_GLOBAL(nm_d4)*)((const NM_GLOBAL(double)*)p + i); o[0] = t.x; o[1] = t.y; o[2] = t.z; }
 NM_FN void gld4(const float* p, int i, float* o) { const nm_f4 t = *(const NM_GLOBAL(nm_f4)*)((const NM_GLOBAL(float)*)p + i); o[0] = t.x; o[1] = t.y; o[2] = t.z; o[3] = t.w; }
@@ -332,6 +344,9 @@
 template <class T> NM_FN V<T> gldv(const T* p, const V<int>& i) { return ldsv(p, i); }
 template <class T> NM_FN void gstv(T* p, const V<int>& i, const V<T>& v, const VB& m) { stsv(p, i, v, m); }
 template <class T> NM_FN void gstv(T* p, const V<int>& i, T v, const VB& m) { stsv(p, i, v, m); }
+template <bool S, class T> NM_FN V<T> gldx(const T* p, const V<int>& i) { return gldv(p, i); }
+template <bool S, class T> NM_FN void gstx(T* p, const V<int>& i, const V<T>& v, const VB& m) { gstv(p, i, v, m); }
+template <bool S, class T> NM_FN void gstx(T* p, const V<int>& i, T v, const VB& m) { gstv(p, i, v, m); }
 template <class T> NM_FN void gld4(const T* p, const V<int>& i, V<T>* o) { for (int k = 0; k < NM_WAVE; k++) for (int c = 0; c < 4; c++) o[c].v[k] = p[i.v[k] + c]; }
 template <class T> NM_FN V<int> to_int(const V<T>& a) { V<int> r; for (int i = 0; i < NM_WAVE; i++) r.v[i] = (int)a.v[i]; return r; }
 template <class T> NM_FN void gld3(const T* p, const V<int>& i, V<T>* o) { for (int k = 0; k < NM_WAVE; k++) for (int c = 0; c < 3; c++) o[c].v[k] = p[i.v[k] + c]; }
```

Measured after the change: 86.58 million env-steps/s (median of 6 runs). 1.03x the previous value.
